# wpeebles/gangealing

Hardware: NVIDIA H100
Metric: gangealing_train_images_per_sec_256 (higher is better)
Workload: dtype f32

## Files before the change

gangealing_b200/_lib.py:

```python
import ctypes
import os

import torch

_HERE = os.path.dirname(os.path.abspath(__file__))
LIB_PATH = os.path.join(_HERE, "libgg_b200.so")

GG_F32, GG_F16, GG_BF16 = 0, 1, 2
PAD_MODES = {"zeros": 0, "border": 1, "reflection": 2}

_c = ctypes
_P, _I, _L, _F = _c.c_void_p, _c.c_int, _c.c_int64, _c.c_float

SIGNATURES = {
    "gg_version": (_I, []),
    "gg_last_error": (_c.c_char_p, []),
    "gg_sm_count": (_I, []),
    "gg_fused_bias_act": (_I, [_P, _P, _P, _P, _I, _I, _I, _F, _F, _L, _L, _L, _P]),
    "gg_noise_bias_act": (_I, [_P, _P, _P, _P, _P, _P, _I, _F, _F, _L, _L, _L, _P]),
    "gg_channel_scale_workspace": (_L, [_L, _L]),
    "gg_channel_scale": (_I, [_P, _P, _P, _P, _P, _P, _I, _L, _L, _P]),
    "gg_bias_act_backward_workspace": (_L, [_L, _L, _L]),
    "gg_bias_act_backward": (_I, [_P, _P, _P, _P, _P, _I, _F, _F, _L, _L, _L, _P]),
    "gg_upfirdn2d": (_I, [_P, _P, _P, _I, _L] + [_I] * 12 + [_P]),
    "gg_blur_noise_bias_act": (_I, [_P] * 7 + [_I, _L, _L] + [_I] * 9 + [_F, _F, _P]),
    "gg_mipmap_pyramid_elems": (_L, [_L, _I, _I, _I]),
    "gg_mipmap_build": (_I, [_P, _P, _I, _L, _I, _I, _I, _P]),
    "gg_mipmap_build_backward": (_I, [_P, _P, _L, _I, _I, _I, _P]),
    "gg_mipmap_warp_forward": (_I, [_P] * 5 + [_I, _L] + [_I] * 6 + [_F, _F, _I, _P]),
    "gg_warp_sample_indices": (_I, [_P, _P, _L, _I, _I, _I, _I, _F, _F, _I, _P]),
    "gg_stn_sample_forward": (_I, [_P] * 11 + [_I, _I, _L] + [_I] * 9 + [_F, _F, _I, _P]),
    "gg_mipmap_warp_lerp_forward": (_I, [_P] * 5 + [_L, _P, _P, _I, _I, _L] + [_I] * 6 + [_F, _F, _I, _P]),
    "gg_mipmap_warp_lerp_mean": (_I, [_P] * 4 + [_L, _P, _P, _I, _I, _L] + [_I] * 6 + [_F, _F, _I, _I, _P]),
    "gg_track_points_lerp": (_I, [_P] * 6 + [_I, _L, _L, _I, _I, _I, _P]),
    "gg_modconv_wsq": (_I, [_P, _P, _I, _I, _I, _P]),
    "gg_modconv_demod": (_I, [_P, _P, _P, _F, _F, _I, _I, _I, _P]),
    "gg_modconv_demod_batched": (_I, [_I, _P, _P, _P, _P, _P, _P, _F, _I, _P]),
    "gg_modconv_modulate": (_I, [_P, _P, _P, _P, _F, _I, _I, _I, _I, _I, _P]),
    "gg_noise_bias_act_nhwc": (_I, [_P] * 6 + [_I, _F, _F, _L, _I, _L, _P]),
    "gg_nhwc_rowwise_workspace": (_L, [_L, _I, _L]),
    "gg_channel_scale_nhwc": (_I, [_P] * 6 + [_I, _L, _I, _L, _P]),
    "gg_bias_act_backward_nhwc": (_I, [_P] * 5 + [_I, _F, _F, _L, _I, _L, _P]),
    "gg_blur_nhwc_workspace": (_L, [_I, _L] + [_I] * 9),
    "gg_blur_nhwc": (_I, [_P] * 12 + [_I, _L] + [_I] * 12 + [_F, _F, _P]),
    "gg_blur_nhwc_mask": (_I, [_P] * 9 + [_I, _L] + [_I] * 11 + [_F, _F, _P]),
    "gg_styled_tail_nhwc": (_I, [_P] * 12 + [_I, _I, _F, _F, _L, _I, _L, _P]),
    "gg_styled_tail_mask_nhwc": (_I, [_P] * 12 + [_I, _I, _F, _F, _L, _I, _L, _P]),
    "gg_styled_tail_backward_mask_nhwc": (_I, [_P] * 7 + [_I, _F, _F, _L, _I, _L, _P]),
    "gg_styled_tail_backward_workspace": (_L, [_I, _L, _I, _L]),
    "gg_styled_tail_backward_nhwc": (_I, [_P] * 12 + [_I, _F, _F, _L, _I, _L, _L, _P]),
    "gg_tent_downsample_forward": (_I, [_P] * 4 + [_L, _I, _I, _I, _I, _P]),
    "gg_tent_downsample_backward": (_I, [_P] * 4 + [_L, _I, _I, _I, _I, _P]),
    "gg_feature_distance_workspace": (_L, [_L, _I, _L]),
    "gg_feature_distance_forward": (_I, [_P] * 5 + [_I, _L, _I, _L, _F, _P]),
    "gg_feature_distance_backward": (_I, [_P] * 6 + [_I, _L, _I, _L, _F, _P]),
    "gg_bias_relu_pool_nhwc_forward": (_I, [_P, _P, _P, _P, _I, _L, _I, _I, _I, _P]),
    "gg_bias_relu_pool_nhwc_backward": (_I, [_P, _P, _P, _P, _I, _L, _I, _I, _I, _P]),
    "gg_to_rgb_nhwc_workspace": (_L, [_L, _I, _L]),
    "gg_to_rgb_nhwc_forward": (_I, [_P] * 5 + [_L, _I, _L, _P]),
    "gg_to_rgb_nhwc_backward": (_I, [_P] * 6 + [_L, _I, _L, _P]),
    "gg_nn_argmin_workspace": (_L, [_L, _L]),
    "gg_nn_argmin": (_I, [_P, _P, _P, _P, _L, _L, _I, _P]),
    "gg_splat2d_lookup_forward": (_I, [_P] * 8 + [_L, _L, _I, _I, _I, _I, _I, _F, _F, _I, _P]),
    "gg_scale_cast_multi": (_I, [_P, _P, _P, _I, _I, _P]),
    "gg_adam_ema_step": (_I, [_P, _P, _P, _I, _I, _P, _c.c_double, _c.c_double, _c.c_double, _c.c_double, _P]),
    "gg_tv_loss_workspace": (_L, [_L, _I, _I]),
    "gg_tv_loss_forward": (_I, [_P, _P, _P, _L, _I, _I, _P]),
    "gg_tv_loss_backward": (_I, [_P, _P, _P, _L, _I, _I, _P]),
    "gg_splat2d_workspace": (_L, [_L, _I, _I, _I]),
    "gg_splat2d_forward": (_I, [_P] * 6 + [_L, _L, _I, _I, _I, _I, _P]),
    "gg_splat_composite_grid_workspace": (_L, [_L, _L, _I, _I]),
    "gg_splat_composite_grid": (_I, [_P, _P, _L, _P, _P, _P, _P, _F, _F, _L, _L, _L, _I, _I, _I, _I, _I, _I, _P]),
    "gg_flow_compose_forward": (_I, [_P] * 7 + [_L, _I, _I, _I, _P]),
    "gg_flow_compose_backward": (_I, [_P] * 10 + [_L, _I, _I, _I, _P]),
    "gg_mipmap_warp_backward": (_I, [_P] * 7 + [_I, _L] + [_I] * 6 + [_F, _F, _I, _P]),
    "gg_laplacian_blend_workspace": (_L, [_L, _I, _I, _I, _I, _I]),
    "gg_laplacian_blend_forward": (_I, [_P] * 6 + [_L, _I, _I, _I, _I, _I, _P]),
    "gg_laplacian_blend_backward": (_I, [_P] * 9 + [_L, _I, _I, _I, _I, _I, _P]),
    "gg_tv_per_sample": (_I, [_P, _P, _L, _I, _I, _P]),
    "gg_pck_transfer_workspace": (_L, [_L, _L, _I]),
    "gg_pck_transfer": (_I, [_P] * 14 + [_L, _L, _I, _I, _I, _I, _I, _P]),
    "gg_batch_gram": (_I, [_P, _P, _P, _P, _L, _I, _P]),
    "gg_flow_image_grid": (_I, [_P, _P, _P, _L, _I, _I, _I, _I, _P]),
    "gg_image_grid": (_I, [_P, _P, _P, _L, _I, _I, _I, _I, _P]),
    "gg_cluster_accumulate": (_I, [_P] * 5 + [_L, _I, _I, _I, _I, _I] + [_L] * 6 + [_I, _P]),
}

_dll = None
CALLS = 0


def load():
    global _dll
    if _dll is None:
        if not os.path.exists(LIB_PATH):
            raise RuntimeError(
                "libgg_b200.so is missing (%s): build it with `python -m gangealing_b200.build` "
                "(there is no CPU/PyTorch fallback for these ops)" % LIB_PATH)
        dll = ctypes.CDLL(LIB_PATH)
        for name, (res, args) in SIGNATURES.items():
            fn = getattr(dll, name)
            fn.restype = res
            fn.argtypes = args
        _dll = dll
    return _dll


def check(rc, what):
    global CALLS
    CALLS += 1
    if rc != 0:
        msg = load().gg_last_error().decode("utf-8", "replace")
        raise RuntimeError("%s failed (%d): %s" % (what, rc, msg))


def dtype_code(t):
    d = t.dtype
    if d == torch.float32:
        return GG_F32
    if d == torch.float16:
        return GG_F16
    if d == torch.bfloat16:
        return GG_BF16
    raise RuntimeError("gangealing_b200: dtype %s is not supported (float32/float16/bfloat16)" % d)


def require_cuda(*tensors):
    for t in tensors:
        if t is None:
            continue
        if not t.is_cuda:
            raise RuntimeError("gangealing_b200 ops run on CUDA tensors only (got a %s tensor); "
                               "the CPU restatement lives in oracle/ and is test infrastructure" % t.device.type)
        if t.device.index != torch.cuda.current_device():
            raise RuntimeError("gangealing_b200: tensor lives on %s but the current device is cuda:%d; wrap the call in "
                               "`with torch.cuda.device(tensor.device):`" % (t.device, torch.cuda.current_device()))


def ptr(t):
    return None if t is None else t.data_ptr()


def is_nhwc(t):
    return (t.dim() == 4 and t.dtype in (torch.float32, torch.bfloat16) and t.shape[1] > 1 and t.shape[2] * t.shape[3] > 1
            and t.is_contiguous(memory_format=torch.channels_last) and not t.is_contiguous())


def nhwc_vec(t):
    return 8 if t.dtype == torch.bfloat16 else 4


def aligned16(t):
    return t.data_ptr() % 16 == 0


def dense_f32(t):
    if t.dtype != torch.float32 or not t.is_contiguous():
        t = t.float().contiguous()
    return t if aligned16(t) else t.clone()


def tensor_cache(t):
    stamp = (t._version, t.data_ptr(), t.device, t.dtype)
    ent = getattr(t, "_gg_cache", None)
    if ent is None or ent[0] != stamp:
        ent = (stamp, {})
        try:
            t._gg_cache = ent
        except Exception:
            pass
    return ent[1]


def filter_is_separable(kernel):
    memo = tensor_cache(kernel)
    v = memo.get("separable")
    if v is None:
        k = kernel.detach().float().cpu()
        big = k.abs().max()
        if big == 0:
            v = True
        else:
            i0, j0 = divmod(int(k.abs().argmax()), k.shape[1])
            v = bool((k - torch.outer(k[:, j0], k[i0, :]) / k[i0, j0]).abs().max() <= 1e-6 * big)
        memo["separable"] = v
    return v


def flipped_filter(kernel):
    memo = tensor_cache(kernel)
    f = memo.get("flipped")
    if f is None:
        f = torch.flip(kernel.detach(), [0, 1])
        fm = tensor_cache(f)
        fm["flipped"] = kernel.detach()
        if "separable" in memo:
            fm["separable"] = memo["separable"]
        memo["flipped"] = f
    return f


def invalidate(t):
    try:
        t._gg_cache = None
    except Exception:
        pass


def stream():
    return torch.cuda.current_stream().cuda_stream


def sm_count():
    return load().gg_sm_count()


def ship_table(slot, payload):
    capturing = torch.cuda.is_current_stream_capturing()
    ev = slot.get("event")
    if ev is not None and not capturing:
        ev.synchronize()
    slot["host"].copy_(payload)
    slot["dev"].copy_(slot["host"], non_blocking=True)
    if capturing:
        slot["event"] = None
    else:
        ev = torch.cuda.Event()
        ev.record()
        slot["event"] = ev
```

gangealing_b200/csrc/common.cuh:

```cuda
#pragma once
#include <cuda_bf16.h>
#include <cuda_fp16.h>
#include <cuda_runtime.h>
#include <stdint.h>

#include <cstdarg>
#include <cstdio>

#include "../../include/gg_b200.h"

namespace gg {

inline char* err_buf() {
  static thread_local char buf[512] = {0};
  return buf;
}
inline int fail(int code, const char* fmt, ...) {
  va_list ap;
  va_start(ap, fmt);
  vsnprintf(err_buf(), 512, fmt, ap);
  va_end(ap);
  return code;
}
inline int cuda_fail(cudaError_t e, const char* what) {
  return fail(GG_ERR_CUDA, "%s: %s", what, cudaGetErrorString(e));
}
#define GG_CHECK_LAUNCH(what)                               \
  do {                                                      \
    cudaError_t e__ = cudaPeekAtLastError();                \
    if (e__ != cudaSuccess) {                               \
      (void)cudaGetLastError();                             \
      return ::gg::cuda_fail(e__, what);                    \
    }                                                       \
  } while (0)

#define GG_DISPATCH_CASE_(code_, type_, ...) \
  case code_: { using T_ = type_; __VA_ARGS__; break; }
#define GG_DISPATCH_T(dtype_, who_, ...)                                                                             \
  switch (dtype_) {                                                                                                  \
    GG_DISPATCH_CASE_(GG_F32, float, __VA_ARGS__)                                                                    \
    GG_DISPATCH_CASE_(GG_BF16, __nv_bfloat16, __VA_ARGS__)                                                           \
    default: return ::gg::fail(GG_ERR_UNSUPPORTED, "%s: dtype %d not supported (fp32 or bf16)", who_, dtype_);       \
  }
#define GG_DISPATCH_T16(dtype_, who_, ...)                                                                           \
  switch (dtype_) {                                                                                                  \
    GG_DISPATCH_CASE_(GG_F32, float, __VA_ARGS__)                                                                    \
    GG_DISPATCH_CASE_(GG_F16, __half, __VA_ARGS__)                                                                   \
    GG_DISPATCH_CASE_(GG_BF16, __nv_bfloat16, __VA_ARGS__)                                                           \
    default: return ::gg::fail(GG_ERR_UNSUPPORTED, "%s: dtype %d not supported (fp32, fp16 or bf16)", who_, dtype_); \
  }

int sm_count();

inline bool aligned16(const void* p) { return (reinterpret_cast<uintptr_t>(p) & 15u) == 0; }
inline bool aligned8(const void* p) { return (reinterpret_cast<uintptr_t>(p) & 7u) == 0; }

struct DeviceOnce {
  unsigned long long mask[2] = {0ull, 0ull};
  int dev = 0;
  bool needed() {
    if (cudaGetDevice(&dev) != cudaSuccess || dev < 0 || dev >= 128) return true;
    return ((__atomic_load_n(&mask[dev >> 6], __ATOMIC_ACQUIRE) >> (dev & 63)) & 1ull) == 0ull;
  }
  void done() {
    if (dev >= 0 && dev < 128) __atomic_fetch_or(&mask[dev >> 6], 1ull << (dev & 63), __ATOMIC_RELEASE);
  }
};

template <typename T> struct Cvt;
template <> struct Cvt<float> {
  static __device__ __forceinline__ float to_f(float v) { return v; }
  static __device__ __forceinline__ float from_f(float v) { return v; }
};
template <> struct Cvt<__half> {
  static __device__ __forceinline__ float to_f(__half v) { return __half2float(v); }
  static __device__ __forceinline__ __half from_f(float v) { return __float2half_rn(v); }
};
template <> struct Cvt<__nv_bfloat16> {
  static __device__ __forceinline__ float to_f(__nv_bfloat16 v) { return __bfloat162float(v); }
  static __device__ __forceinline__ __nv_bfloat16 from_f(float v) { return __float2bfloat16_rn(v); }
};

template <typename T> struct alignas(16) Vec16 {
  static constexpr int N = 16 / sizeof(T);
  T v[N];
};

template <typename T>
__device__ __forceinline__ Vec16<T> ld_vec_stream(const T* p) {
  Vec16<T> r;
  uint4 u;
  asm volatile("ld.global.nc.L1::no_allocate.v4.u32 {%0,%1,%2,%3}, [%4];"
               : "=r"(u.x), "=r"(u.y), "=r"(u.z), "=r"(u.w)
               : "l"(p));
  *reinterpret_cast<uint4*>(&r) = u;
  return r;
}
template <typename T>
__device__ __forceinline__ void st_vec_stream(T* p, const Vec16<T>& r) {
  const uint4 u = *reinterpret_cast<const uint4*>(&r);
  asm volatile("st.global.L1::no_allocate.v4.u32 [%0], {%1,%2,%3,%4};" ::"l"(p), "r"(u.x), "r"(u.y),
               "r"(u.z), "r"(u.w)
               : "memory");
}

template <typename T> struct ChanVec;
template <> struct ChanVec<float> {
  static constexpr int V = 4;
  static __device__ __forceinline__ void unpack(const uint4& u, float (&f)[4]) {
    f[0] = __uint_as_float(u.x); f[1] = __uint_as_float(u.y); f[2] = __uint_as_float(u.z); f[3] = __uint_as_float(u.w);
  }
  static __device__ __forceinline__ uint4 pack(const float (&f)[4]) {
    return make_uint4(__float_as_uint(f[0]), __float_as_uint(f[1]), __float_as_uint(f[2]), __float_as_uint(f[3]));
  }
};
template <> struct ChanVec<__nv_bfloat16> {
  static constexpr int V = 8;
  static __device__ __forceinline__ void unpack(const uint4& u, float (&f)[8]) {
    f[0] = __uint_as_float(u.x << 16); f[1] = __uint_as_float(u.x & 0xffff0000u);
    f[2] = __uint_as_float(u.y << 16); f[3] = __uint_as_float(u.y & 0xffff0000u);
    f[4] = __uint_as_float(u.z << 16); f[5] = __uint_as_float(u.z & 0xffff0000u);
    f[6] = __uint_as_float(u.w << 16); f[7] = __uint_as_float(u.w & 0xffff0000u);
  }
  static __device__ __forceinline__ uint32_t pack2(float lo, float hi) {
    const __nv_bfloat162 h = __floats2bfloat162_rn(lo, hi);
    return *reinterpret_cast<const uint32_t*>(&h);
  }
  static __device__ __forceinline__ uint4 pack(const float (&f)[8]) {
    return make_uint4(pack2(f[0], f[1]), pack2(f[2], f[3]), pack2(f[4], f[5]), pack2(f[6], f[7]));
  }
};
__device__ __forceinline__ uint4 ldg_stream16(const void* p) {
  uint4 u;
  asm volatile("ld.global.nc.L1::no_allocate.v4.u32 {%0,%1,%2,%3}, [%4];" : "=r"(u.x), "=r"(u.y), "=r"(u.z), "=r"(u.w) : "l"(p));
  return u;
}
__device__ __forceinline__ void stg_stream16(void* p, const uint4& u) {
  asm volatile("st.global.L1::no_allocate.v4.u32 [%0], {%1,%2,%3,%4};" ::"l"(p), "r"(u.x), "r"(u.y), "r"(u.z), "r"(u.w) : "memory");
}

template <typename T> struct SignFloor { static constexpr float v = 0.f; };
template <> struct SignFloor<__nv_bfloat16> { static constexpr float v = 0x1p-134f; };

template <typename T, int V>
__device__ __forceinline__ uint32_t sign_bits(const float (&o)[V]) {
  uint32_t m = 0u;
#pragma unroll
  for (int k = 0; k < V; ++k) m |= (o[k] > SignFloor<T>::v ? 1u : 0u) << k;
  return m;
}
template <int V>
__device__ __forceinline__ uint32_t sign_word(uint32_t bits, int cq, unsigned lanes) {
  constexpr int L = 32 / V;
  uint32_t w = bits << (V * (cq & (L - 1)));
#pragma unroll
  for (int m = L / 2; m >= 1; m >>= 1) w |= __shfl_xor_sync(lanes, w, m);
  return w;
}
template <int V>
__device__ __forceinline__ uint32_t sign_load(const uint32_t* px, int cq) {
  return __ldg(px + (cq * V >> 5)) >> (cq * V & 31);
}

__device__ __forceinline__ float warp_sum(float v) {
#pragma unroll
  for (int o = 16; o > 0; o >>= 1) v += __shfl_xor_sync(0xffffffffu, v, o);
  return v;
}

__device__ __forceinline__ uint32_t smem_u32(const void* p) {
  return static_cast<uint32_t>(__cvta_generic_to_shared(p));
}
__device__ __forceinline__ void mbar_init(uint64_t* bar, uint32_t count) {
  asm volatile("mbarrier.init.shared::cta.b64 [%0], %1;" ::"r"(smem_u32(bar)), "r"(count));
}
__device__ __forceinline__ void mbar_fence_init() {
  asm volatile("fence.mbarrier_init.release.cluster;" ::: "memory");
}
__device__ __forceinline__ void mbar_expect_tx(uint64_t* bar, uint32_t bytes) {
  asm volatile("mbarrier.arrive.expect_tx.shared::cta.b64 _, [%0], %1;" ::"r"(smem_u32(bar)),
               "r"(bytes)
               : "memory");
}
__device__ __forceinline__ void mbar_wait(uint64_t* bar, uint32_t parity) {
  uint32_t done;
  uint32_t spins = 0;
  do {
    if (++spins == (1u << 28)) __trap();
    asm volatile(
        "{\n\t"
        ".reg .pred p;\n\t"
        "mbarrier.try_wait.parity.shared::cta.b64 p, [%1], %2;\n\t"
        "selp.u32 %0, 1, 0, p;\n\t"
        "}"
        : "=r"(done)
        : "r"(smem_u32(bar)), "r"(parity)
        : "memory");
  } while (!done);
}
__device__ __forceinline__ void tma_bulk_g2s(void* dst_smem, const void* src_gmem, uint32_t bytes,
                                             uint64_t* bar) {
  asm volatile(
      "cp.async.bulk.shared::cluster.global.mbarrier::complete_tx::bytes [%0], [%1], %2, [%3];" ::"r"(
          smem_u32(dst_smem)),
      "l"(src_gmem), "r"(bytes), "r"(smem_u32(bar))
      : "memory");
}

}
```

gangealing_b200/csrc/nhwc.cu:

```cuda
#include <cuda.h>

#include "common.cuh"
#include "nhwc_reduce.cuh"

namespace gg {
namespace {

constexpr int kT = 256;

template <typename T>
__global__ void __launch_bounds__(kT)
noise_bias_act_nhwc_kernel(T* __restrict__ out, const T* __restrict__ x, const float* __restrict__ noise,
                           const float* __restrict__ noise_weight, const float* __restrict__ bias,
                           const float* __restrict__ row_scale, float alpha, float gain, int64_t n_vec, int cv,
                           int64_t hw) {
  constexpr int V = ChanVec<T>::V;
  const float nw = noise ? (noise_weight ? __ldg(noise_weight) : 1.f) : 0.f;
  const int64_t base = (static_cast<int64_t>(blockIdx.x) * 4) * kT + threadIdx.x;
  uint4 xv[4];
#pragma unroll
  for (int u = 0; u < 4; ++u) {
    const int64_t v = base + static_cast<int64_t>(u) * kT;
    if (v < n_vec) xv[u] = ldg_stream16(x + v * V);
  }
#pragma unroll
  for (int u = 0; u < 4; ++u) {
    const int64_t v = base + static_cast<int64_t>(u) * kT;
    if (v < n_vec) {
      int64_t pix, n = 0;
      int cq;
      if (n_vec <= 0xffffffffLL) {
        const unsigned v32 = static_cast<unsigned>(v), p32 = v32 / static_cast<unsigned>(cv);
        cq = static_cast<int>(v32 - p32 * static_cast<unsigned>(cv));
        pix = p32;
        if (row_scale) n = p32 / static_cast<unsigned>(hw);
      } else {
        pix = v / cv;
        cq = static_cast<int>(v - pix * cv);
        if (row_scale) n = pix / hw;
      }
      const float nz = noise ? nw * __ldg(noise + pix) : 0.f;
      float xf[V], o[V];
      ChanVec<T>::unpack(xv[u], xf);
#pragma unroll
      for (int q = 0; q < V / 4; ++q) {
        const float4 b = bias ? __ldg(reinterpret_cast<const float4*>(bias) + cq * (V / 4) + q) : make_float4(0.f, 0.f, 0.f, 0.f);
        const float4 r = row_scale ? __ldg(reinterpret_cast<const float4*>(row_scale + n * cv * V) + cq * (V / 4) + q)
                                   : make_float4(1.f, 1.f, 1.f, 1.f);
        const float bb[4] = {b.x, b.y, b.z, b.w}, rr[4] = {r.x, r.y, r.z, r.w};
#pragma unroll
        for (int k = 0; k < 4; ++k) {
          const float t = fmaf(xf[4 * q + k], rr[k], bb[k]) + nz;
          o[4 * q + k] = (t > 0.f ? t : t * alpha) * gain;
        }
      }
      stg_stream16(out + v * V, ChanVec<T>::pack(o));
    }
  }
}

template <typename T, int MODE>
__global__ void __launch_bounds__(kT)
rowwise_nhwc_kernel(T* __restrict__ out, float* __restrict__ partial, const T* __restrict__ x,
                    const T* __restrict__ y, const float* __restrict__ s, float alpha, float gain, int cv,
                    int64_t hw, int chunk, int chunks_per_sample) {
  constexpr int V = ChanVec<T>::V;
  extern __shared__ float red[];
  const int64_t n = blockIdx.x / chunks_per_sample;
  const int ck = blockIdx.x - n * chunks_per_sample;
  const int64_t p0 = static_cast<int64_t>(ck) * chunk, p1 = min(p0 + chunk, hw);
  const int lanes_p = kT / cv > 0 ? kT / cv : 1;
  float acc[V];
#pragma unroll
  for (int k = 0; k < V; ++k) acc[k] = 0.f;
  const int cq = threadIdx.x % cv;
  const int pl = threadIdx.x / cv;
  if (pl < lanes_p) {
    float sv[V];
#pragma unroll
    for (int k = 0; k < V; ++k) sv[k] = (MODE == 0) ? __ldg(s + n * cv * V + cq * V + k) : 1.f;
    const bool has_y = (MODE == 1) || y != nullptr;
    auto body = [&](const uint4 xr, const uint4 yr, int64_t off) {
      float xf[V], yf[V], o[V];
      ChanVec<T>::unpack(xr, xf);
      ChanVec<T>::unpack(yr, yf);
#pragma unroll
      for (int k = 0; k < V; ++k) {
        if (MODE == 0) {
          o[k] = xf[k] * sv[k];
          if (has_y) acc[k] = fmaf(xf[k], yf[k], acc[k]);
        } else {
          o[k] = (yf[k] > 0.f ? xf[k] : xf[k] * alpha) * gain;
          acc[k] += o[k];
        }
      }
      *reinterpret_cast<uint4*>(out + off) = ChanVec<T>::pack(o);
    };
    const uint4 zero = make_uint4(0u, 0u, 0u, 0u);
    int64_t p = p0 + pl;
    for (; p + 3 * lanes_p < p1; p += 4 * lanes_p) {
      uint4 xv[4], yv[4];
      int64_t off[4];
#pragma unroll
      for (int u = 0; u < 4; ++u) {
        off[u] = ((n * hw + p + u * lanes_p) * cv + cq) * V;
        xv[u] = ldg_stream16(x + off[u]);
      }
#pragma unroll
      for (int u = 0; u < 4; ++u) yv[u] = has_y ? ldg_stream16(y + off[u]) : zero;
#pragma unroll
      for (int u = 0; u < 4; ++u) body(xv[u], yv[u], off[u]);
    }
    for (; p < p1; p += lanes_p) {
      const int64_t off = ((n * hw + p) * cv + cq) * V;
      const uint4 xv = ldg_stream16(x + off);
      const uint4 yv = has_y ? ldg_stream16(y + off) : zero;
      body(xv, yv, off);
    }
  }
  if (partial) {
    const int C = cv * V;
    if (pl < lanes_p) {
#pragma unroll
      for (int q = 0; q < V / 4; ++q)
        reinterpret_cast<float4*>(red + pl * C + cq * V)[q] = make_float4(acc[4 * q], acc[4 * q + 1], acc[4 * q + 2], acc[4 * q + 3]);
    }
    __syncthreads();
    for (int c = threadIdx.x; c < C; c += kT) {
      float t = 0.f;
      for (int l = 0; l < lanes_p; ++l) t += red[l * C + c];
      partial[static_cast<int64_t>(blockIdx.x) * C + c] = t;
    }
  }
}

__global__ void __launch_bounds__(kT)
to_rgb_nhwc_fwd_kernel(float* __restrict__ out, const float* __restrict__ x, const float* __restrict__ wm,
                       const float* __restrict__ bias, const float* __restrict__ skip, int c4, int64_t hw, int chunk,
                       int chunks_per_sample) {
  extern __shared__ __align__(16) float wsm[];
  const int64_t n = blockIdx.x / chunks_per_sample;
  const int ck = blockIdx.x - n * chunks_per_sample;
  const int64_t p0 = static_cast<int64_t>(ck) * chunk, p1 = min(p0 + chunk, hw);
  {
    const float4* src = reinterpret_cast<const float4*>(wm + n * 3 * c4 * 4);
    float4* dst = reinterpret_cast<float4*>(wsm);
    for (int i = threadIdx.x; i < 3 * c4; i += kT) dst[i] = __ldg(src + i);
  }
  __syncthreads();
  const float4* w4 = reinterpret_cast<const float4*>(wsm);
  const int l = threadIdx.x & 7, grp = threadIdx.x >> 3;
  const bool vec_ok = (hw & 3) == 0;
  const unsigned gmask = 0xffu << (threadIdx.x & 24);
  for (int64_t pb = p0 + grp * 4; pb < p1; pb += (kT / 8) * 4) {
    float acc[4][3];
#pragma unroll
    for (int u = 0; u < 4; ++u) acc[u][0] = acc[u][1] = acc[u][2] = 0.f;
    const float4* xp[4];
#pragma unroll
    for (int u = 0; u < 4; ++u) {
      const int64_t pu = min(pb + u, p1 - 1);
      xp[u] = reinterpret_cast<const float4*>(x + (n * hw + pu) * c4 * 4);
    }
    for (int q = l; q < c4; q += 8) {
      float4 xv[4];
#pragma unroll
      for (int u = 0; u < 4; ++u) xv[u] = __ldcs(xp[u] + q);
      const float4 w0 = w4[q], w1 = w4[c4 + q], w2 = w4[2 * c4 + q];
#pragma unroll
      for (int u = 0; u < 4; ++u) {
        acc[u][0] = fmaf(xv[u].x, w0.x, fmaf(xv[u].y, w0.y, fmaf(xv[u].z, w0.z, fmaf(xv[u].w, w0.w, acc[u][0]))));
        acc[u][1] = fmaf(xv[u].x, w1.x, fmaf(xv[u].y, w1.y, fmaf(xv[u].z, w1.z, fmaf(xv[u].w, w1.w, acc[u][1]))));
        acc[u][2] = fmaf(xv[u].x, w2.x, fmaf(xv[u].y, w2.y, fmaf(xv[u].z, w2.z, fmaf(xv[u].w, w2.w, acc[u][2]))));
      }
    }
#pragma unroll
    for (int m = 4; m >= 1; m >>= 1)
#pragma unroll
      for (int u = 0; u < 4; ++u)
#pragma unroll
        for (int o = 0; o < 3; ++o) acc[u][o] += __shfl_xor_sync(gmask, acc[u][o], m);
    if (l < 3) {
      const int o = l;
      float r[4];
#pragma unroll
      for (int u = 0; u < 4; ++u) r[u] = (o == 0 ? acc[u][0] : o == 1 ? acc[u][1] : acc[u][2]) + (bias ? __ldg(bias + o) : 0.f);
      const int64_t off = (n * 3 + o) * hw + pb;
      if (vec_ok && pb + 3 < p1) {
        if (skip) {
          const float4 sk = __ldg(reinterpret_cast<const float4*>(skip + off));
          r[0] += sk.x; r[1] += sk.y; r[2] += sk.z; r[3] += sk.w;
        }
        *reinterpret_cast<float4*>(out + off) = make_float4(r[0], r[1], r[2], r[3]);
      } else {
#pragma unroll
        for (int u = 0; u < 4; ++u)
          if (pb + u < p1) out[off + u] = r[u] + (skip ? __ldg(skip + off + u) : 0.f);
      }
    }
  }
}

__global__ void __launch_bounds__(kT)
to_rgb_nhwc_bwd_kernel(float* __restrict__ gx, float* __restrict__ partial, const float* __restrict__ g,
                       const float* __restrict__ x, const float* __restrict__ wm, int c4, int64_t hw, int chunk,
                       int chunks_per_sample) {
  extern __shared__ float red[];
  const int64_t n = blockIdx.x / chunks_per_sample;
  const int ck = blockIdx.x - n * chunks_per_sample;
  const int64_t p0 = static_cast<int64_t>(ck) * chunk, p1 = min(p0 + chunk, hw);
  const int lanes_p = kT / c4 > 0 ? kT / c4 : 1;
  const int cq = threadIdx.x % c4, pl = threadIdx.x / c4;
  float4 a0 = make_float4(0.f, 0.f, 0.f, 0.f), a1 = a0, a2 = a0;
  if (pl < lanes_p) {
    const float4* wp = reinterpret_cast<const float4*>(wm + n * 3 * c4 * 4);
    const float4 w0 = __ldg(wp + cq), w1 = __ldg(wp + c4 + cq), w2 = __ldg(wp + 2 * c4 + cq);
    const float* g0 = g + n * 3 * hw;
    auto body = [&](int64_t p, const float4 xv, float s0, float s1, float s2) {
      float4 o;
      o.x = fmaf(w2.x, s2, fmaf(w1.x, s1, w0.x * s0)); o.y = fmaf(w2.y, s2, fmaf(w1.y, s1, w0.y * s0));
      o.z = fmaf(w2.z, s2, fmaf(w1.z, s1, w0.z * s0)); o.w = fmaf(w2.w, s2, fmaf(w1.w, s1, w0.w * s0));
      if (gx) *reinterpret_cast<float4*>(gx + ((n * hw + p) * c4 + cq) * 4) = o;
      a0.x = fmaf(s0, xv.x, a0.x); a0.y = fmaf(s0, xv.y, a0.y); a0.z = fmaf(s0, xv.z, a0.z); a0.w = fmaf(s0, xv.w, a0.w);
      a1.x = fmaf(s1, xv.x, a1.x); a1.y = fmaf(s1, xv.y, a1.y); a1.z = fmaf(s1, xv.z, a1.z); a1.w = fmaf(s1, xv.w, a1.w);
      a2.x = fmaf(s2, xv.x, a2.x); a2.y = fmaf(s2, xv.y, a2.y); a2.z = fmaf(s2, xv.z, a2.z); a2.w = fmaf(s2, xv.w, a2.w);
    };
    const float4 zero = make_float4(0.f, 0.f, 0.f, 0.f);
    int64_t p = p0 + pl;
    for (; p + 3 * lanes_p < p1; p += 4 * lanes_p) {
      float4 xv[4];
      float s[4][3];
#pragma unroll
      for (int u = 0; u < 4; ++u) {
        const int64_t pu = p + u * lanes_p;
        xv[u] = partial ? __ldcs(reinterpret_cast<const float4*>(x + ((n * hw + pu) * c4 + cq) * 4)) : zero;
        s[u][0] = __ldg(g0 + pu); s[u][1] = __ldg(g0 + hw + pu); s[u][2] = __ldg(g0 + 2 * hw + pu);
      }
#pragma unroll
      for (int u = 0; u < 4; ++u) body(p + u * lanes_p, xv[u], s[u][0], s[u][1], s[u][2]);
    }
    for (; p < p1; p += lanes_p) {
      const float4 xv = partial ? __ldcs(reinterpret_cast<const float4*>(x + ((n * hw + p) * c4 + cq) * 4)) : zero;
      body(p, xv, __ldg(g0 + p), __ldg(g0 + hw + p), __ldg(g0 + 2 * hw + p));
    }
  }
  if (partial) {
    float4* r4 = reinterpret_cast<float4*>(red);
    if (pl < lanes_p) {
      r4[(pl * 3 + 0) * c4 + cq] = a0; r4[(pl * 3 + 1) * c4 + cq] = a1; r4[(pl * 3 + 2) * c4 + cq] = a2;
    }
    __syncthreads();
    for (int i = threadIdx.x; i < 3 * c4; i += kT) {
      float4 t = make_float4(0.f, 0.f, 0.f, 0.f);
      for (int q = 0; q < lanes_p; ++q) {
        const float4 v = r4[q * 3 * c4 + i];
        t.x += v.x; t.y += v.y; t.z += v.z; t.w += v.w;
      }
      reinterpret_cast<float4*>(partial + static_cast<int64_t>(blockIdx.x) * 3 * c4 * 4)[i] = t;
    }
  }
}

template <typename T> struct BlurGeom {
  static constexpr int V = ChanVec<T>::V;
  static constexpr int CB = 8 * V;
  static constexpr int COLS = (V == 4) ? 2 : 1;
  static constexpr int BX = 32 * COLS;
  static constexpr int TW = BX + 3;
  static constexpr int STAGE_ELEMS = 4 * TW * CB;
};
constexpr int kRY = 4;
constexpr int kNS = 3;

struct BlurNhwcParams {
  int n, c, in_h, in_w, out_h, out_w;
  int pad_x0, pad_y0;
  int seg_rows;
  int act;
  float alpha, gain;
};

__device__ __forceinline__ void tma_load_4d(void* smem_dst, const CUtensorMap* tmap, int c0, int x0, int y0, int n0,
                                            uint64_t* bar) {
  asm volatile(
      "cp.async.bulk.tensor.4d.shared::cluster.global.tile.mbarrier::complete_tx::bytes [%0], [%1, {%2, %3, %4, %5}], [%6];"
      ::"r"(smem_u32(smem_dst)), "l"(tmap), "r"(c0), "r"(x0), "r"(y0), "r"(n0), "r"(smem_u32(bar))
      : "memory");
}

template <typename T, int MODE, bool SEP, bool FAST = false>
__global__ void __launch_bounds__(kT, 2)
blur_nhwc_kernel(T* __restrict__ out, T* __restrict__ out2, const __grid_constant__ CUtensorMap tmap,
                 const float* __restrict__ filt, int kh, int kw, const float* __restrict__ noise,
                 const float* __restrict__ noise_weight, const float* __restrict__ bias,
                 const float* __restrict__ row_scale, const float* __restrict__ scale2, const T* __restrict__ mul,
                 float* __restrict__ partial, BlurNhwcParams p) {
  using G = BlurGeom<T>;
  constexpr int V = G::V, CB = G::CB, COLS = G::COLS, BX = G::BX, TW = G::TW;
  constexpr bool FUSED = MODE == 1 || MODE == 3;
  constexpr bool MASK = MODE == 3;
  extern __shared__ __align__(128) unsigned char tiles_raw[];
  T* tiles = reinterpret_cast<T*>(tiles_raw);
  __shared__ uint64_t full_bar[kNS];
  const int tid = threadIdx.x;
  const int cq = tid & 7;
  const int xg = tid >> 3;
  const int chunks = p.c / CB;
  const int bx = blockIdx.x / chunks, cc = blockIdx.x - bx * chunks;
  const int n = blockIdx.z;
  const int oy0 = blockIdx.y * p.seg_rows;
  const int rows_out = min(p.seg_rows, p.out_h - oy0);
  const int x_out0 = bx * BX;
  const int c0 = cc * CB;
  const int iy0 = oy0 - p.pad_y0, ix0 = x_out0 - p.pad_x0;
  const int rows_in = rows_out + 3;
  const int n_stage_iters = (rows_in + kRY - 1) / kRY;
  constexpr uint32_t kStageBytes = G::STAGE_ELEMS * sizeof(T);

  if (tid == 0) {
#pragma unroll
    for (int s = 0; s < kNS; ++s) mbar_init(&full_bar[s], 1);
    mbar_fence_init();
  }
  __syncthreads();
  if (tid == 0) {
#pragma unroll
    for (int s = 0; s < kNS - 1; ++s)
      if (s < n_stage_iters) {
        mbar_expect_tx(&full_bar[s], kStageBytes);
        tma_load_4d(tiles + s * G::STAGE_ELEMS, &tmap, c0, ix0, iy0 + s * kRY, n, &full_bar[s]);
      }
  }

  float kf[4][4];
#pragma unroll
  for (int a = 0; a < 4; ++a)
#pragma unroll
    for (int b = 0; b < 4; ++b)
      kf[a][b] = (a < kh && b < kw) ? __ldg(filt + (kh - 1 - a) * kw + (kw - 1 - b)) : 0.f;
  float ku[4], kv[4];
  {
    int a0 = 0, b0 = 0;
    float big = 0.f;
#pragma unroll
    for (int a = 0; a < 4; ++a)
#pragma unroll
      for (int b = 0; b < 4; ++b)
        if (fabsf(kf[a][b]) > big) { big = fabsf(kf[a][b]); a0 = a; b0 = b; }
    float piv = 1.f;
#pragma unroll
    for (int a = 0; a < 4; ++a)
#pragma unroll
      for (int b = 0; b < 4; ++b)
        if (a == a0 && b == b0) piv = kf[a][b];
    const float inv = big > 0.f ? 1.f / piv : 0.f;
#pragma unroll
    for (int a = 0; a < 4; ++a) {
      float col = 0.f;
#pragma unroll
      for (int b = 0; b < 4; ++b) if (b == b0) col = kf[a][b];
      ku[a] = col * inv;
    }
#pragma unroll
    for (int b = 0; b < 4; ++b) {
      float row = 0.f;
#pragma unroll
      for (int a = 0; a < 4; ++a) if (a == a0) row = kf[a][b];
      kv[b] = row;
    }
  }

  float bq[V], rq[V], sq[V], dacc[V];
#pragma unroll
  for (int k = 0; k < V; ++k) { bq[k] = 0.f; rq[k] = 1.f; sq[k] = 1.f; dacc[k] = 0.f; }
  float nw = 0.f;
  const int64_t nc0 = static_cast<int64_t>(n) * p.c + c0 + cq * V;
  if (MODE != 0) {
    if (row_scale) {
#pragma unroll
      for (int k = 0; k < V; ++k) rq[k] = __ldg(row_scale + nc0 + k);
    }
  }
  if (FUSED) {
    if (bias) {
#pragma unroll
      for (int k = 0; k < V; ++k) bq[k] = __ldg(bias + c0 + cq * V + k);
    }
    if (scale2) {
#pragma unroll
      for (int k = 0; k < V; ++k) sq[k] = __ldg(scale2 + nc0 + k);
    }
    nw = noise ? (noise_weight ? __ldg(noise_weight) : 1.f) : 0.f;
  }
  constexpr bool fast = FUSED && FAST;
  const float neg = (p.act == 3) ? p.alpha : 1.f;
  if (fast) {
#pragma unroll
    for (int k = 0; k < V; ++k) { rq[k] *= p.gain; bq[k] *= p.gain; }
    nw *= p.gain;
  }
  const int xo = x_out0 + COLS * xg;
  const int64_t row_stride = static_cast<int64_t>(p.out_w) * p.c;
  const int64_t obase = ((static_cast<int64_t>(n) * p.out_h + oy0) * p.out_w + xo) * p.c + c0 + cq * V;
  int64_t ocur = obase - 3 * row_stride;
  bool okc[COLS];
#pragma unroll
  for (int j = 0; j < COLS; ++j) okc[j] = xo + j < p.out_w;
  float nzn[kRY][COLS];
#pragma unroll
  for (int rr = 0; rr < kRY; ++rr)
#pragma unroll
    for (int j = 0; j < COLS; ++j) nzn[rr][j] = 0.f;
  const float* noise_base = noise ? noise + (static_cast<int64_t>(n) * p.out_h + oy0) * p.out_w + xo : nullptr;
  auto fetch_noise = [&](int it_) {
#pragma unroll
    for (int rr = 0; rr < kRY; ++rr) {
      const int ro = it_ * kRY + rr - 3;
#pragma unroll
      for (int j = 0; j < COLS; ++j) nzn[rr][j] = 0.f;
      if (ro >= 0 && ro < rows_out) {
        const float* np_ = noise_base + static_cast<int64_t>(ro) * p.out_w;
#pragma unroll
        for (int j = 0; j < COLS; ++j)
          if (okc[j]) nzn[rr][j] = __ldg(np_ + j);
      }
    }
  };
  if (FUSED && noise) fetch_noise(0);

  uint4 mcur[COLS], mnext[COLS];
#pragma unroll
  for (int j = 0; j < COLS; ++j) mcur[j] = mnext[j] = make_uint4(0u, 0u, 0u, 0u);
  auto fetch_mul = [&](int ro_) {
    if (ro_ >= 0 && ro_ < rows_out) {
      const int64_t mo = obase + ro_ * row_stride;
#pragma unroll
      for (int j = 0; j < COLS; ++j)
        if (okc[j]) mnext[j] = __ldg(reinterpret_cast<const uint4*>(mul + mo + static_cast<int64_t>(j) * p.c));
    }
  };
  if (MODE == 2 && mul) { fetch_mul(-3 + 3); }

  float hwin[SEP ? 4 : 1][COLS][V];
  float rwin[SEP ? 1 : 4][COLS + 3][V];
  int r_in = 0;
  for (int it = 0; it < n_stage_iters; ++it) {
    const int stage = it % kNS;
    if (tid == 0) {
      const int nxt = it + kNS - 1;
      if (nxt < n_stage_iters) {
        const int ns = nxt % kNS;
        asm volatile("fence.proxy.async.shared::cta;" ::: "memory");
        mbar_expect_tx(&full_bar[ns], kStageBytes);
        tma_load_4d(tiles + ns * G::STAGE_ELEMS, &tmap, c0, ix0, iy0 + nxt * kRY, n, &full_bar[ns]);
      }
    }
    float nzc[kRY][COLS];
#pragma unroll
    for (int rr = 0; rr < kRY; ++rr)
#pragma unroll
      for (int j = 0; j < COLS; ++j) nzc[rr][j] = nzn[rr][j];
    if (FUSED && noise && it + 1 < n_stage_iters) fetch_noise(it + 1);
    if (MODE == 2 && mul && it + 1 < n_stage_iters) {
#pragma unroll
      for (int rr = 0; rr < kRY; ++rr) {
        const int ro = (it + 1) * kRY + rr - 3;
        if (ro >= 0 && ro < rows_out) {
          const T* mp = mul + obase + ro * row_stride;
#pragma unroll
          for (int j = 0; j < COLS; ++j)
            if (okc[j]) asm volatile("prefetch.global.L2 [%0];" ::"l"(mp + static_cast<int64_t>(j) * p.c));
        }
      }
    }
    mbar_wait(&full_bar[stage], static_cast<uint32_t>((it / kNS) & 1));
    const T* st = tiles + stage * G::STAGE_ELEMS;
#pragma unroll
    for (int rr = 0; rr < kRY; ++rr, ++r_in, ocur += row_stride) {
      if (MODE == 2 && mul) {
#pragma unroll
        for (int j = 0; j < COLS; ++j) mcur[j] = mnext[j];
        fetch_mul(r_in - 3 + 1);
      }
      const uint4* rowp = reinterpret_cast<const uint4*>(st + (rr * TW + COLS * xg) * CB) + cq;
      float q[COLS + 3][V];
#pragma unroll
      for (int i = 0; i < COLS + 3; ++i) ChanVec<T>::unpack(rowp[i * 8], q[i]);
      if constexpr (SEP) {
#pragma unroll
        for (int j = 0; j < COLS; ++j)
#pragma unroll
          for (int k = 0; k < V; ++k) {
            float h = __fmul_rn(kv[0], q[j][k]);
            h = __fmaf_rn(kv[1], q[j + 1][k], h);
            h = __fmaf_rn(kv[2], q[j + 2][k], h);
            h = __fmaf_rn(kv[3], q[j + 3][k], h);
            hwin[rr][j][k] = h;
          }
      } else {
#pragma unroll
        for (int i = 0; i < COLS + 3; ++i)
#pragma unroll
          for (int k = 0; k < V; ++k) rwin[rr][i][k] = q[i][k];
      }
      const int ro = r_in - 3;
      if (ro >= 0 && ro < rows_out) {
#pragma unroll
        for (int j = 0; j < COLS; ++j) {
          float a4[V];
          if constexpr (SEP) {
#pragma unroll
            for (int k = 0; k < V; ++k) {
              float a = __fmul_rn(ku[0], hwin[(rr + 1) & 3][j][k]);
              a = __fmaf_rn(ku[1], hwin[(rr + 2) & 3][j][k], a);
              a = __fmaf_rn(ku[2], hwin[(rr + 3) & 3][j][k], a);
              a = __fmaf_rn(ku[3], hwin[rr][j][k], a);
              a4[k] = a;
            }
          } else {
#pragma unroll
            for (int k = 0; k < V; ++k) a4[k] = 0.f;
#pragma unroll
            for (int a = 0; a < 4; ++a)
#pragma unroll
              for (int b = 0; b < 4; ++b)
#pragma unroll
                for (int k = 0; k < V; ++k) a4[k] = fmaf(kf[a][b], rwin[(rr + 1 + a) & 3][j + b][k], a4[k]);
          }
          const int64_t ooff = ocur + j * p.c;
          if (FUSED) {
            const float nzj = nw * nzc[rr][j];
            float o2[V];
#pragma unroll
            for (int k = 0; k < V; ++k) {
              float t = __fmaf_rn(a4[k], rq[k], __fadd_rn(bq[k], nzj));
              const float tn = __fmul_rn(t, neg);
              if (fast) t = fmaxf(t, tn);
              else t = (t > 0.f ? t : tn) * p.gain;
              a4[k] = t;
              o2[k] = __fmul_rn(t, sq[k]);
            }
            uint32_t word = 0u;
            if (MASK) word = sign_word<V>(sign_bits<T>(a4), cq, 0xffffffffu);
            if (okc[j]) {
              if (MASK) {
                if ((cq * V & 31) == 0) reinterpret_cast<uint32_t*>(out)[ooff >> 5] = word;
              } else if (out) {
                *reinterpret_cast<uint4*>(out + ooff) = ChanVec<T>::pack(a4);
              }
              if (out2) *reinterpret_cast<uint4*>(out2 + ooff) = ChanVec<T>::pack(o2);
            }
          } else if (MODE == 2) {
            if (okc[j]) {
              if (mul) {
                float mf[V];
                ChanVec<T>::unpack(mcur[j], mf);
#pragma unroll
                for (int k = 0; k < V; ++k) dacc[k] = fmaf(a4[k], mf[k], dacc[k]);
              }
#pragma unroll
              for (int k = 0; k < V; ++k) a4[k] *= rq[k];
              *reinterpret_cast<uint4*>(out + ooff) = ChanVec<T>::pack(a4);
            }
          } else {
            if (okc[j]) *reinterpret_cast<uint4*>(out + ooff) = ChanVec<T>::pack(a4);
          }
        }
      }
    }
    __syncthreads();
  }
  if (MODE == 2 && partial) {
    float* red = reinterpret_cast<float*>(tiles_raw);
#pragma unroll
    for (int k = 0; k < V; ++k) red[xg * CB + cq * V + k] = dacc[k];
    __syncthreads();
    if (tid < CB) {
      float t = 0.f;
#pragma unroll 8
      for (int g = 0; g < 32; ++g) t += red[g * CB + tid];
      const int64_t K = static_cast<int64_t>(gridDim.x / chunks) * gridDim.y;
      const int64_t kidx = static_cast<int64_t>(bx) * gridDim.y + blockIdx.y;
      partial[(static_cast<int64_t>(n) * K + kidx) * p.c + c0 + tid] = t;
    }
  }
}

typedef CUresult (*EncodeTiledFn)(CUtensorMap*, CUtensorMapDataType, cuuint32_t, void*, const cuuint64_t*, const cuuint64_t*,
                                  const cuuint32_t*, const cuuint32_t*, CUtensorMapInterleave, CUtensorMapSwizzle,
                                  CUtensorMapL2promotion, CUtensorMapFloatOOBfill);

inline EncodeTiledFn encode_fn() {
  static EncodeTiledFn fn = nullptr;
  if (!fn) {
    void* p = nullptr;
    cudaDriverEntryPointQueryResult q;
    if (cudaGetDriverEntryPoint("cuTensorMapEncodeTiled", &p, cudaEnableDefault, &q) == cudaSuccess &&
        q == cudaDriverEntryPointSuccess)
      fn = reinterpret_cast<EncodeTiledFn>(p);
  }
  return fn;
}

inline int grid1(int64_t total, int per_cta) {
  int64_t g = (total + per_cta - 1) / per_cta;
  return static_cast<int>(g > 0 ? g : 1);
}

}
}

using namespace gg;

extern "C" {

static inline int vec_of(int dtype) { return dtype == GG_BF16 ? 8 : 4; }

int gg_noise_bias_act_nhwc(void* out, const void* x, const float* noise, const float* noise_weight, const float* bias,
                           const float* row_scale, int dtype, float alpha, float scale, int64_t N, int C, int64_t HW,
                           void* stream) {
  if (N < 0 || C < 0 || HW < 0) return fail(GG_ERR_BAD_ARG, "noise_bias_act_nhwc: negative size");
  if (dtype != GG_F32 && dtype != GG_BF16) return fail(GG_ERR_UNSUPPORTED, "noise_bias_act_nhwc: dtype %d not supported", dtype);
  const int64_t numel = N * HW * C;
  if (numel == 0) return GG_OK;
  const int V = vec_of(dtype);
  if (C % V != 0) return fail(GG_ERR_UNSUPPORTED, "noise_bias_act_nhwc: C must be a multiple of %d", V);
  if (!out || !x) return fail(GG_ERR_BAD_ARG, "noise_bias_act_nhwc: null tensor");
  if (!aligned16(bias) || !aligned16(row_scale))
    return fail(GG_ERR_BAD_ARG, "noise_bias_act_nhwc: bias and row_scale must be 16-byte aligned");
  const int64_t n_vec = numel / V;
  const int64_t grid = (n_vec + 4 * kT - 1) / (4 * kT);
  if (grid > 0x7fffffffLL) return fail(GG_ERR_BAD_ARG, "noise_bias_act_nhwc: tensor too large");
  GG_DISPATCH_T(dtype, "noise_bias_act_nhwc",
                (noise_bias_act_nhwc_kernel<T_><<<static_cast<unsigned>(grid), kT, 0, static_cast<cudaStream_t>(stream)>>>(
                    static_cast<T_*>(out), static_cast<const T_*>(x), noise, noise_weight, bias, row_scale, alpha, scale,
                    n_vec, C / V, HW)));
  GG_CHECK_LAUNCH("noise_bias_act_nhwc launch");
  return GG_OK;
}

static int64_t rowwise_chunk(int64_t N, int cv, int64_t HW) {
  const int lanes_p = kT / cv > 0 ? kT / cv : 1;
  const int64_t target = 8LL * sm_count();
  int64_t k = (target + N - 1) / N;
  const int64_t kmax = (HW + 4 * lanes_p - 1) / (4 * lanes_p);
  if (k > kmax) k = kmax;
  if (k < 1) k = 1;
  return (HW + k - 1) / k;
}

int64_t gg_nhwc_rowwise_workspace(int64_t N, int C, int64_t HW) {
  if (N <= 0 || C <= 0 || HW <= 0 || C % 4 != 0) return 0;
  const int64_t chunk = rowwise_chunk(N, C / 4, HW);
  const int64_t chunk8 = (C % 8 == 0) ? rowwise_chunk(N, C / 8, HW) : chunk;
  const int64_t k = (HW + (chunk < chunk8 ? chunk : chunk8) - 1) / (chunk < chunk8 ? chunk : chunk8);
  return N * k * C * static_cast<int64_t>(sizeof(float));
}

static int launch_rowwise(int mode, void* out, float* dst, void* workspace, const void* x, const void* y, const float* s,
                          int dtype, float alpha, float gain, int64_t N, int C, int64_t HW, bool per_sample, void* stream) {
  if (N < 0 || C < 0 || HW < 0) return fail(GG_ERR_BAD_ARG, "nhwc rowwise: negative size");
  if (dtype != GG_F32 && dtype != GG_BF16) return fail(GG_ERR_UNSUPPORTED, "nhwc rowwise: dtype %d not supported", dtype);
  if (N * HW * C == 0) {
    const int64_t sums = (per_sample ? N : 1) * C;
    if (dst && sums > 0) {
      cudaError_t e = cudaMemsetAsync(dst, 0, sums * sizeof(float), static_cast<cudaStream_t>(stream));
      if (e != cudaSuccess) return cuda_fail(e, "nhwc rowwise memset");
    }
    return GG_OK;
  }
  const int V = vec_of(dtype);
  if (C % V != 0 || C / V > kT) return fail(GG_ERR_UNSUPPORTED, "nhwc rowwise: C must be a multiple of %d and <= %d", V, V * kT);
  if (!out || !x) return fail(GG_ERR_BAD_ARG, "nhwc rowwise: null tensor");
  if (dst && !workspace) return fail(GG_ERR_BAD_ARG, "nhwc rowwise: reduction needs a workspace");
  const int cv = C / V;
  const int64_t chunk64 = rowwise_chunk(N, cv, HW);
  if (chunk64 > 0x7fffffffLL) return fail(GG_ERR_BAD_ARG, "nhwc rowwise: plane too large");
  const int chunk = static_cast<int>(chunk64);
  const int K = static_cast<int>((HW + chunk - 1) / chunk);
  const int64_t grid = N * K;
  if (grid > 0x7fffffffLL) return fail(GG_ERR_BAD_ARG, "nhwc rowwise: too many CTAs");
  const int lanes_p = kT / cv > 0 ? kT / cv : 1;
  const size_t smem = static_cast<size_t>(lanes_p) * C * sizeof(float);
  float* partial = dst ? static_cast<float*>(workspace) : nullptr;
  auto st = static_cast<cudaStream_t>(stream);
  const unsigned g = static_cast<unsigned>(grid);
  if (mode == 0) {
    GG_DISPATCH_T(dtype, "nhwc rowwise",
                  (rowwise_nhwc_kernel<T_, 0><<<g, kT, smem, st>>>(static_cast<T_*>(out), partial, static_cast<const T_*>(x),
                                                                 dst ? static_cast<const T_*>(y) : nullptr, s, alpha, gain,
                                                                 cv, HW, chunk, K)));
  } else {
    GG_DISPATCH_T(dtype, "nhwc rowwise",
                  (rowwise_nhwc_kernel<T_, 1><<<g, kT, smem, st>>>(static_cast<T_*>(out), partial, static_cast<const T_*>(x),
                                                                 static_cast<const T_*>(y), s, alpha, gain, cv, HW, chunk, K)));
  }
  GG_CHECK_LAUNCH("nhwc rowwise launch");
  if (dst) {
    const int64_t rows = per_sample ? N : 1;
    const int kk = per_sample ? K : static_cast<int>(N * K);
    nhwc_finish_kernel<<<static_cast<unsigned>(rows * ((C + 31) / 32)), dim3(32, 32), 0, st>>>(dst, partial, rows, kk, C);
    GG_CHECK_LAUNCH("nhwc finish launch");
  }
  return GG_OK;
}

int gg_channel_scale_nhwc(void* out, float* row_dot, void* workspace, const void* x, const void* y, const float* s,
                          int dtype, int64_t N, int C, int64_t HW, void* stream) {
  if (!s) return fail(GG_ERR_BAD_ARG, "channel_scale_nhwc: null scale");
  if (row_dot && !y) return fail(GG_ERR_BAD_ARG, "channel_scale_nhwc: row_dot needs y");
  return launch_rowwise(0, out, row_dot, workspace, x, y, s, dtype, 0.f, 1.f, N, C, HW, true, stream);
}

int gg_bias_act_backward_nhwc(void* gx, float* grad_bias, void* workspace, const void* g, const void* out_saved,
                              int dtype, float alpha, float scale, int64_t N, int C, int64_t HW, void* stream) {
  if (!out_saved) return fail(GG_ERR_BAD_ARG, "bias_act_backward_nhwc: null saved output");
  return launch_rowwise(1, gx, grad_bias, workspace, g, out_saved, nullptr, dtype, alpha, scale, N, C, HW, false, stream);
}

int64_t gg_to_rgb_nhwc_workspace(int64_t N, int C, int64_t HW) { return 3 * gg_nhwc_rowwise_workspace(N, C, HW); }

int gg_to_rgb_nhwc_forward(float* out, const float* x, const float* wm, const float* bias, const float* skip, int64_t N,
                           int C, int64_t HW, void* stream) {
  if (N < 0 || C < 0 || HW < 0) return fail(GG_ERR_BAD_ARG, "to_rgb_nhwc: negative size");
  if (N * HW == 0) return GG_OK;
  if (C < 32 || C % 32 != 0 || C > 1024) return fail(GG_ERR_UNSUPPORTED, "to_rgb_nhwc: C must be a multiple of 32, <= 1024");
  if (!out || !x || !wm) return fail(GG_ERR_BAD_ARG, "to_rgb_nhwc: null tensor");
  if (!aligned16(wm) || (HW % 4 == 0 && (!aligned16(skip) || !aligned16(out))))
    return fail(GG_ERR_BAD_ARG, "to_rgb_nhwc: wm (and skip, out when HW %% 4 == 0) must be 16-byte aligned");
  const int64_t target = 8LL * sm_count();
  int64_t k = (target + N - 1) / N;
  const int64_t kmax = (HW + 127) / 128;
  if (k > kmax) k = kmax;
  if (k < 1) k = 1;
  int64_t chunk = ((HW + k - 1) / k + 127) / 128 * 128;
  if (chunk > 0x7fffff00LL) return fail(GG_ERR_BAD_ARG, "to_rgb_nhwc: plane too large");
  const int K = static_cast<int>((HW + chunk - 1) / chunk);
  const int64_t grid = N * K;
  if (grid > 0x7fffffffLL) return fail(GG_ERR_BAD_ARG, "to_rgb_nhwc: too many CTAs");
  to_rgb_nhwc_fwd_kernel<<<static_cast<unsigned>(grid), kT, static_cast<size_t>(3) * C * sizeof(float),
                           static_cast<cudaStream_t>(stream)>>>(out, x, wm, bias, skip, C / 4, HW, static_cast<int>(chunk), K);
  GG_CHECK_LAUNCH("to_rgb_nhwc forward launch");
  return GG_OK;
}

int gg_to_rgb_nhwc_backward(float* gx, float* gwm, void* workspace, const float* g, const float* x, const float* wm,
                            int64_t N, int C, int64_t HW, void* stream) {
  if (N < 0 || C < 0 || HW < 0) return fail(GG_ERR_BAD_ARG, "to_rgb_nhwc backward: negative size");
  if (N * HW == 0 || C == 0) {
    if (gwm && N * C > 0) {
      cudaError_t e = cudaMemsetAsync(gwm, 0, N * 3 * C * sizeof(float), static_cast<cudaStream_t>(stream));
      if (e != cudaSuccess) return cuda_fail(e, "to_rgb_nhwc backward memset");
    }
    return GG_OK;
  }
  if (C % 4 != 0 || C > 1024) return fail(GG_ERR_UNSUPPORTED, "to_rgb_nhwc backward: C must be a multiple of 4, <= 1024");
  if (!g || !wm || (!gx && !gwm)) return fail(GG_ERR_BAD_ARG, "to_rgb_nhwc backward: null tensor");
  if (gwm && (!x || !workspace)) return fail(GG_ERR_BAD_ARG, "to_rgb_nhwc backward: gwm needs x and a workspace");
  if (!aligned16(wm)) return fail(GG_ERR_BAD_ARG, "to_rgb_nhwc backward: wm must be 16-byte aligned");
  const int c4 = C / 4;
  const int64_t chunk64 = rowwise_chunk(N, c4, HW);
  if (chunk64 > 0x7fffffffLL) return fail(GG_ERR_BAD_ARG, "to_rgb_nhwc backward: plane too large");
  const int chunk = static_cast<int>(chunk64);
  const int K = static_cast<int>((HW + chunk - 1) / chunk);
  const int64_t grid = N * K;
  if (grid > 0x7fffffffLL) return fail(GG_ERR_BAD_ARG, "to_rgb_nhwc backward: too many CTAs");
  const int lanes_p = kT / c4 > 0 ? kT / c4 : 1;
  const size_t smem = static_cast<size_t>(lanes_p) * 3 * C * sizeof(float);
  auto st = static_cast<cudaStream_t>(stream);
  float* partial = gwm ? static_cast<float*>(workspace) : nullptr;
  to_rgb_nhwc_bwd_kernel<<<static_cast<unsigned>(grid), kT, smem, st>>>(gx, partial, g, x, wm, c4, HW, chunk, K);
  GG_CHECK_LAUNCH("to_rgb_nhwc backward launch");
  if (gwm) {
    nhwc_finish_kernel<<<static_cast<unsigned>(N * ((3 * C + 31) / 32)), dim3(32, 32), 0, st>>>(gwm, partial, N, K, 3 * C);
    GG_CHECK_LAUNCH("to_rgb_nhwc finish launch");
  }
  return GG_OK;
}

struct BlurPlan {
  int out_h, out_w, xblocks, chunks, segs, seg_rows;
};
static int blur_plan(BlurPlan* pl, int dtype, int64_t N, int C, int in_h, int in_w, int kernel_h, int kernel_w, int pad_x0,
                     int pad_x1, int pad_y0, int pad_y1) {
  const int V = vec_of(dtype);
  const int CB = 8 * V, BX = (V == 4) ? 64 : 32;
  if (C % CB != 0) return fail(GG_ERR_UNSUPPORTED, "blur_nhwc: C must be a multiple of %d", CB);
  pl->out_h = in_h + pad_y0 + pad_y1 - kernel_h + 1;
  pl->out_w = in_w + pad_x0 + pad_x1 - kernel_w + 1;
  if (pl->out_h < 1 || pl->out_w < 1) return fail(GG_ERR_BAD_ARG, "blur_nhwc: empty output");
  pl->xblocks = (pl->out_w + BX - 1) / BX;
  pl->chunks = C / CB;
  const int64_t base_ctas = static_cast<int64_t>(pl->xblocks) * pl->chunks * (N > 0 ? N : 1);
  int segs = static_cast<int>((2LL * 2 * sm_count() + base_ctas - 1) / base_ctas);
  int seg_rows = (pl->out_h + segs - 1) / segs;
  if (seg_rows < 16) seg_rows = pl->out_h < 16 ? pl->out_h : 16;
  seg_rows = (seg_rows + 3) / 4 * 4;
  pl->seg_rows = seg_rows;
  pl->segs = (pl->out_h + seg_rows - 1) / seg_rows;
  return GG_OK;
}

int64_t gg_blur_nhwc_workspace(int dtype, int64_t N, int C, int in_h, int in_w, int kernel_h, int kernel_w, int pad_x0,
                               int pad_x1, int pad_y0, int pad_y1) {
  BlurPlan pl;
  if (N <= 0 || C <= 0 || (dtype != GG_F32 && dtype != GG_BF16)) return 0;
  if (blur_plan(&pl, dtype, N, C, in_h, in_w, kernel_h, kernel_w, pad_x0, pad_x1, pad_y0, pad_y1) != GG_OK) return 0;
  return N * static_cast<int64_t>(pl.xblocks) * pl.segs * C * static_cast<int64_t>(sizeof(float));
}

}

template <typename T>
static int launch_blur(void* out, void* out2, const void* in, const float* kernel, const float* noise,
                       const float* noise_weight, const float* bias, const float* row_scale, const float* scale2,
                       const void* mul, float* row_dot, void* workspace, int64_t N, int C, int in_h, int in_w, int kernel_h,
                       int kernel_w, int separable, int pad_x0, int pad_x1, int pad_y0, int pad_y1, int mode, int act,
                       float alpha, float scale, void* stream, int dtype, bool out_is_mask) {
  using G = BlurGeom<T>;
  BlurPlan pl;
  int rc = blur_plan(&pl, dtype, N, C, in_h, in_w, kernel_h, kernel_w, pad_x0, pad_x1, pad_y0, pad_y1);
  if (rc != GG_OK) return rc;
  EncodeTiledFn enc = encode_fn();
  if (!enc) return fail(GG_ERR_CUDA, "blur_nhwc: cuTensorMapEncodeTiled is not available from this driver");
  struct MapKey { const void* ptr; int64_t n; int c, h, w, es; };
  struct MapEnt { MapKey key; CUtensorMap map; bool valid; };
  static thread_local MapEnt cache[16] = {};
  static thread_local unsigned cache_next = 0;
  const MapKey key = {in, N, C, in_h, in_w, static_cast<int>(sizeof(T))};
  const CUtensorMap* cached = nullptr;
  for (int i = 0; i < 16 && !cached; ++i)
    if (cache[i].valid && cache[i].key.ptr == key.ptr && cache[i].key.n == key.n && cache[i].key.c == key.c &&
        cache[i].key.h == key.h && cache[i].key.w == key.w && cache[i].key.es == key.es)
      cached = &cache[i].map;
  CUtensorMap tmap;
  if (cached) tmap = *cached;
  const cuuint64_t es = sizeof(T);
  const cuuint64_t gdim[4] = {static_cast<cuuint64_t>(C), static_cast<cuuint64_t>(in_w), static_cast<cuuint64_t>(in_h),
                              static_cast<cuuint64_t>(N)};
  const cuuint64_t gstr[3] = {static_cast<cuuint64_t>(C) * es, static_cast<cuuint64_t>(in_w) * C * es,
                              static_cast<cuuint64_t>(in_h) * in_w * C * es};
  const cuuint32_t box[4] = {G::CB, G::TW, kRY, 1};
  const cuuint32_t estr[4] = {1, 1, 1, 1};
  if (!cached) {
    const CUresult r = enc(&tmap, sizeof(T) == 4 ? CU_TENSOR_MAP_DATA_TYPE_FLOAT32 : CU_TENSOR_MAP_DATA_TYPE_BFLOAT16, 4,
                           const_cast<void*>(in), gdim, gstr, box, estr, CU_TENSOR_MAP_INTERLEAVE_NONE,
                           CU_TENSOR_MAP_SWIZZLE_NONE, CU_TENSOR_MAP_L2_PROMOTION_L2_128B, CU_TENSOR_MAP_FLOAT_OOB_FILL_NONE);
    if (r != CUDA_SUCCESS) return fail(GG_ERR_CUDA, "blur_nhwc: cuTensorMapEncodeTiled failed (%d)", static_cast<int>(r));
    MapEnt& e = cache[cache_next++ % 16];
    e.key = key; e.map = tmap; e.valid = true;
  }
  BlurNhwcParams p;
  p.n = static_cast<int>(N); p.c = C; p.in_h = in_h; p.in_w = in_w; p.out_h = pl.out_h; p.out_w = pl.out_w;
  p.pad_x0 = pad_x0; p.pad_y0 = pad_y0;
  p.act = act; p.alpha = alpha; p.gain = scale;
  p.seg_rows = pl.seg_rows;
  const dim3 grid(static_cast<unsigned>(pl.xblocks * pl.chunks), static_cast<unsigned>(pl.segs), static_cast<unsigned>(N));
  const size_t smem = static_cast<size_t>(kNS) * G::STAGE_ELEMS * sizeof(T);
  static DeviceOnce configured;
  if (configured.needed()) {
    cudaError_t e = cudaSuccess;
    const void* kernels[12] = {reinterpret_cast<const void*>(blur_nhwc_kernel<T, 0, true>),
                              reinterpret_cast<const void*>(blur_nhwc_kernel<T, 0, false>),
                              reinterpret_cast<const void*>(blur_nhwc_kernel<T, 1, true, false>),
                              reinterpret_cast<const void*>(blur_nhwc_kernel<T, 1, false, false>),
                              reinterpret_cast<const void*>(blur_nhwc_kernel<T, 1, true, true>),
                              reinterpret_cast<const void*>(blur_nhwc_kernel<T, 1, false, true>),
                              reinterpret_cast<const void*>(blur_nhwc_kernel<T, 3, true, false>),
                              reinterpret_cast<const void*>(blur_nhwc_kernel<T, 3, false, false>),
                              reinterpret_cast<const void*>(blur_nhwc_kernel<T, 3, true, true>),
                              reinterpret_cast<const void*>(blur_nhwc_kernel<T, 3, false, true>),
                              reinterpret_cast<const void*>(blur_nhwc_kernel<T, 2, true>),
                              reinterpret_cast<const void*>(blur_nhwc_kernel<T, 2, false>)};
    for (int i = 0; i < 12 && e == cudaSuccess; ++i)
      e = cudaFuncSetAttribute(kernels[i], cudaFuncAttributeMaxDynamicSharedMemorySize, static_cast<int>(smem));
    if (e != cudaSuccess) return cuda_fail(e, "blur_nhwc smem opt-in");
    configured.done();
  }
  auto st = static_cast<cudaStream_t>(stream);
  float* partial = (mode == 2 && row_dot) ? static_cast<float*>(workspace) : nullptr;
  const bool fast = scale > 0.f && ((act == 3 && alpha >= 0.f && alpha <= 1.f) || act == 1);
#define GG_BLUR(M_, S_, F_)                                                                                          \
  blur_nhwc_kernel<T, M_, S_, F_><<<grid, kT, smem, st>>>(static_cast<T*>(out), static_cast<T*>(out2), tmap, kernel, kernel_h, \
                                                         kernel_w, noise, noise_weight, bias, row_scale, scale2,     \
                                                         static_cast<const T*>(mul), partial, p)
  if (mode == 1 && out_is_mask) {
    if (fast) { if (separable) GG_BLUR(3, true, true); else GG_BLUR(3, false, true); }
    else { if (separable) GG_BLUR(3, true, false); else GG_BLUR(3, false, false); }
  }
  else if (mode == 1) {
    if (fast) { if (separable) GG_BLUR(1, true, true); else GG_BLUR(1, false, true); }
    else { if (separable) GG_BLUR(1, true, false); else GG_BLUR(1, false, false); }
  }
  else if (mode == 2) { if (separable) GG_BLUR(2, true, false); else GG_BLUR(2, false, false); }
  else { if (separable) GG_BLUR(0, true, false); else GG_BLUR(0, false, false); }
#undef GG_BLUR
  GG_CHECK_LAUNCH("blur_nhwc launch");
  if (partial) {
    const int K = pl.xblocks * pl.segs;
    nhwc_finish_kernel<<<static_cast<unsigned>(N * ((C + 31) / 32)), dim3(32, 32), 0, st>>>(row_dot, partial, N, K, C);
    GG_CHECK_LAUNCH("blur_nhwc finish launch");
  }
  return GG_OK;
}

extern "C" {

int gg_blur_nhwc(void* out, void* out2, const void* in, const float* kernel, const float* noise, const float* noise_weight,
                 const float* bias, const float* row_scale, const float* scale2, const void* mul, float* row_dot,
                 void* workspace, int dtype, int64_t N, int C, int in_h, int in_w, int kernel_h, int kernel_w, int separable,
                 int pad_x0, int pad_x1, int pad_y0, int pad_y1, int mode, int act, float alpha, float scale, void* stream) {
  if (N < 0 || C < 0 || in_h < 1 || in_w < 1) return fail(GG_ERR_BAD_ARG, "blur_nhwc: bad shape");
  if (kernel_h < 1 || kernel_w < 1 || kernel_h > 4 || kernel_w > 4) return fail(GG_ERR_UNSUPPORTED, "blur_nhwc: filter must be <= 4x4");
  if (mode < 0 || mode > 2) return fail(GG_ERR_BAD_ARG, "blur_nhwc: mode must be 0 (blur), 1 (fused tail) or 2 (adjoint epilogue)");
  if (act != 1 && act != 3) return fail(GG_ERR_UNSUPPORTED, "blur_nhwc: act must be 1 or 3");
  if (dtype != GG_F32 && dtype != GG_BF16) return fail(GG_ERR_UNSUPPORTED, "blur_nhwc: dtype %d not supported (fp32 or bf16)", dtype);
  if (N == 0 || C == 0) return GG_OK;
  if (!in || !kernel) return fail(GG_ERR_BAD_ARG, "blur_nhwc: null tensor");
  if (mode == 1 ? (!out && !out2) : !out) return fail(GG_ERR_BAD_ARG, "blur_nhwc: null output");
  if (mode != 1 && out2) return fail(GG_ERR_BAD_ARG, "blur_nhwc: out2 belongs to the fused tail (mode 1)");
  if (mode == 2 && row_dot && (!mul || !workspace)) return fail(GG_ERR_BAD_ARG, "blur_nhwc: row_dot needs `mul` and a workspace");
  if (N > 65535) return fail(GG_ERR_UNSUPPORTED, "blur_nhwc: batch > 65535");
  if (mode == 0) { noise = nullptr; noise_weight = nullptr; bias = nullptr; row_scale = nullptr; scale2 = nullptr; }
  GG_DISPATCH_T(dtype, "blur_nhwc",
                return launch_blur<T_>(out, out2, in, kernel, noise, noise_weight, bias, row_scale, scale2, mul, row_dot,
                                       workspace, N, C, in_h, in_w, kernel_h, kernel_w, separable, pad_x0, pad_x1, pad_y0,
                                       pad_y1, mode, act, alpha, scale, stream, dtype, false));
  return GG_OK;
}

int gg_blur_nhwc_mask(void* mask, void* out2, const void* in, const float* kernel, const float* noise,
                      const float* noise_weight, const float* bias, const float* row_scale, const float* scale2, int dtype,
                      int64_t N, int C, int in_h, int in_w, int kernel_h, int kernel_w, int separable, int pad_x0, int pad_x1,
                      int pad_y0, int pad_y1, int act, float alpha, float scale, void* stream) {
  if (N < 0 || C < 0 || in_h < 1 || in_w < 1) return fail(GG_ERR_BAD_ARG, "blur_nhwc_mask: bad shape");
  if (kernel_h < 1 || kernel_w < 1 || kernel_h > 4 || kernel_w > 4) return fail(GG_ERR_UNSUPPORTED, "blur_nhwc_mask: filter must be <= 4x4");
  if (act != 1 && act != 3) return fail(GG_ERR_UNSUPPORTED, "blur_nhwc_mask: act must be 1 or 3");
  if (dtype != GG_F32 && dtype != GG_BF16) return fail(GG_ERR_UNSUPPORTED, "blur_nhwc_mask: dtype %d not supported (fp32 or bf16)", dtype);
  if (N == 0 || C == 0) return GG_OK;
  if (!in || !kernel) return fail(GG_ERR_BAD_ARG, "blur_nhwc_mask: null tensor");
  if (!mask) return fail(GG_ERR_BAD_ARG, "blur_nhwc_mask: null mask");
  if (out2 && !scale2) return fail(GG_ERR_BAD_ARG, "blur_nhwc_mask: out2 needs scale2");
  if (N > 65535) return fail(GG_ERR_UNSUPPORTED, "blur_nhwc_mask: batch > 65535");
  GG_DISPATCH_T(dtype, "blur_nhwc_mask",
                return launch_blur<T_>(mask, out2, in, kernel, noise, noise_weight, bias, row_scale, scale2, nullptr, nullptr,
                                       nullptr, N, C, in_h, in_w, kernel_h, kernel_w, separable, pad_x0, pad_x1, pad_y0,
                                       pad_y1, 1, act, alpha, scale, stream, dtype, true));
  return GG_OK;
}

}
```

gangealing_b200/op/nhwc.py:

```python
import torch

from .. import _lib

CL = torch.channels_last

TIMING = None


def elementwise_ok(t):
    return _lib.is_nhwc(t) and t.shape[1] % _lib.nhwc_vec(t) == 0 and _lib.aligned16(t)


def rowwise_ok(t):
    return elementwise_ok(t) and t.shape[1] // _lib.nhwc_vec(t) <= 256


def blur_ok(t, kh, kw, up=(1, 1), down=(1, 1)):
    return (_lib.is_nhwc(t) and t.shape[1] % (8 * _lib.nhwc_vec(t)) == 0 and kh <= 4 and kw <= 4
            and up == (1, 1) and down == (1, 1) and _lib.aligned16(t))


def _f32(t, numel=None):
    if t is None:
        return None
    t = _lib.dense_f32(t.detach())
    if numel is not None and t.numel() != numel:
        raise RuntimeError("channels-last op: expected %d fp32 values, got %d" % (numel, t.numel()))
    return t


def noise_plane(noise, n, h, w):
    if noise is None:
        return None
    noise = noise.detach()
    if noise.numel() != n * h * w:
        noise = noise.expand(n, 1, h, w)
    return noise.float().contiguous()


def sign_mask_empty(n, c, h, w, device):
    if c % 32:
        raise RuntimeError("sign mask: C = %d is not a multiple of 32" % c)
    return torch.empty((n, h, w, c // 32), dtype=torch.int32, device=device)


def blur(x, kernel, pad, mode=0, noise=None, noise_weight=None, bias=None, row_scale=None, scale2=None, want_out=True,
         want_out2=False, mul=None, want_dot=False, negative_slope=0.2, gain=1.0, act=3, want_mask=False):
    n, c, in_h, in_w = x.shape
    taps = kernel.detach()
    if taps.dtype != torch.float32 or not taps.is_contiguous():
        taps = taps.float().contiguous()
    kh, kw = taps.shape
    out_h = in_h + pad[2] + pad[3] - kh + 1
    out_w = in_w + pad[0] + pad[1] - kw + 1
    if out_h < 1 or out_w < 1:
        raise RuntimeError("blur: empty output (%d x %d)" % (out_h, out_w))
    lib = _lib.load()
    code = _lib.dtype_code(x)

    def empty():
        return torch.empty((n, c, out_h, out_w), dtype=x.dtype, device=x.device, memory_format=CL)
    if want_mask and mode != 1:
        raise RuntimeError("blur: the sign mask belongs to the fused tail (mode 1)")
    if want_mask:
        out = sign_mask_empty(n, c, out_h, out_w, x.device)
    else:
        out = empty() if (want_out or mode != 1) else None
    out2 = empty() if (mode == 1 and want_out2) else None
    nz = noise_plane(noise, n, out_h, out_w) if mode == 1 else None
    dot = ws = None
    if mode == 2 and want_dot:
        if (mul is None or mul.shape != (n, c, out_h, out_w) or mul.dtype != x.dtype or not mul.is_contiguous(memory_format=CL)
                or not _lib.aligned16(mul)):
            raise RuntimeError("blur (adjoint epilogue): `mul` must be a 16-byte-aligned channels-last tensor of the output's "
                               "shape and dtype")
        dot = torch.empty((n, c), dtype=torch.float32, device=x.device)
        nbytes = lib.gg_blur_nhwc_workspace(code, n, c, in_h, in_w, kh, kw, pad[0], pad[1], pad[2], pad[3])
        ws = torch.empty(max(1, nbytes // 4), dtype=torch.float32, device=x.device)
    timed = TIMING is not None and mode == 1
    if timed:
        ev0, ev1 = torch.cuda.Event(enable_timing=True), torch.cuda.Event(enable_timing=True)
        ev0.record()
    nw, b, rs, s2 = _f32(noise_weight, 1), _f32(bias, c), _f32(row_scale, n * c), _f32(scale2, n * c)
    sep = 1 if _lib.filter_is_separable(kernel) else 0
    if want_mask:
        rc = lib.gg_blur_nhwc_mask(out.data_ptr(), _lib.ptr(out2), x.data_ptr(), taps.data_ptr(), _lib.ptr(nz), _lib.ptr(nw),
                                   _lib.ptr(b), _lib.ptr(rs), _lib.ptr(s2), code, n, c, in_h, in_w, kh, kw, sep, pad[0],
                                   pad[1], pad[2], pad[3], act, negative_slope, gain, _lib.stream())
    else:
        rc = lib.gg_blur_nhwc(_lib.ptr(out), _lib.ptr(out2), x.data_ptr(), taps.data_ptr(), _lib.ptr(nz),
                              _lib.ptr(nw), _lib.ptr(b), _lib.ptr(rs),
                              _lib.ptr(s2), _lib.ptr(mul if dot is not None else None), _lib.ptr(dot), _lib.ptr(ws),
                              code, n, c, in_h, in_w, kh, kw, sep, pad[0], pad[1],
                              pad[2], pad[3], mode, act, negative_slope, gain, _lib.stream())
    _lib.check(rc, "gg_blur_nhwc_mask" if want_mask else "gg_blur_nhwc")
    if timed:
        ev1.record()
        es = x.element_size()
        writes = (out is not None and not want_mask) + (out2 is not None)
        TIMING.append((ev0, ev1, es * n * c * (in_h * in_w + writes * out_h * out_w) + (4 * n * out_h * out_w if nz is not None else 0)
                       + (out.numel() * 4 if want_mask else 0)
                       + 4 * ((2 + (scale2 is not None)) * c + 1 + kh * kw)))
    return out, out2, dot


def noise_bias_act(x, noise, noise_weight, bias, row_scale, negative_slope, gain):
    n, c, h, w = x.shape
    out = torch.empty_like(x)
    nz, nw, b, rs = noise_plane(noise, n, h, w), _f32(noise_weight, 1), _f32(bias, c), _f32(row_scale, n * c)
    rc = _lib.load().gg_noise_bias_act_nhwc(out.data_ptr(), x.data_ptr(), _lib.ptr(nz), _lib.ptr(nw), _lib.ptr(b),
                                            _lib.ptr(rs), _lib.dtype_code(x), negative_slope, gain, n, c, h * w,
                                            _lib.stream())
    _lib.check(rc, "gg_noise_bias_act_nhwc")
    return out


def bias_act_backward(g, out_saved, negative_slope, gain, want_bias_grad):
    n, c, h, w = out_saved.shape
    lib = _lib.load()
    gx = torch.empty_like(out_saved)
    grad_bias = ws = None
    if want_bias_grad:
        grad_bias = torch.empty(c, dtype=torch.float32, device=g.device)
        ws = torch.empty(max(1, lib.gg_nhwc_rowwise_workspace(n, c, h * w) // 4), dtype=torch.float32, device=g.device)
    rc = lib.gg_bias_act_backward_nhwc(gx.data_ptr(), _lib.ptr(grad_bias), _lib.ptr(ws), g.data_ptr(), out_saved.data_ptr(),
                                       _lib.dtype_code(out_saved), negative_slope, gain, n, c, h * w, _lib.stream())
    _lib.check(rc, "gg_bias_act_backward_nhwc")
    return gx, grad_bias


def channel_scale(x, s, y=None):
    n, c, h, w = x.shape
    lib = _lib.load()
    out = torch.empty_like(x)
    dot = ws = None
    if y is not None:
        dot = torch.empty((n, c), dtype=torch.float32, device=x.device)
        ws = torch.empty(max(1, lib.gg_nhwc_rowwise_workspace(n, c, h * w) // 4), dtype=torch.float32, device=x.device)
    sc = _f32(s, n * c)
    rc = lib.gg_channel_scale_nhwc(out.data_ptr(), _lib.ptr(dot), _lib.ptr(ws), x.data_ptr(), _lib.ptr(y), sc.data_ptr(),
                                   _lib.dtype_code(x), n, c, h * w, _lib.stream())
    _lib.check(rc, "gg_channel_scale_nhwc")
    return out, dot


def _activation_like(t, like, who, name):
    if t is not None and (t.shape != like.shape or t.dtype != like.dtype or not t.is_contiguous(memory_format=CL)
                          or not _lib.aligned16(t)):
        raise RuntimeError("%s: %s must be a 16-byte-aligned channels-last tensor of the activation's shape and dtype"
                           % (who, name))


def _rgb_grad_ok(g_rgb, n, h, w, who):
    if g_rgb is not None and (g_rgb.shape != (n, 3, h, w) or g_rgb.dtype != torch.float32 or not g_rgb.is_contiguous()):
        raise RuntimeError("%s: g_rgb must be a dense fp32 (N, 3, H, W) tensor" % who)


def styled_tail(raw, noise, noise_weight, bias, demod, s_next, wm, rgb_bias, skip, want_out, negative_slope, gain, act=3,
                want_mask=False):
    _activation_like(raw, raw, "styled_tail", "raw")
    n, c, h, w = raw.shape
    if want_mask:
        out = sign_mask_empty(n, c, h, w, raw.device)
    else:
        out = torch.empty_like(raw) if want_out else None
    xs = torch.empty_like(raw) if s_next is not None else None
    rgb = torch.empty((n, 3, h, w), dtype=torch.float32, device=raw.device) if wm is not None else None
    sk = None
    if skip is not None and rgb is not None:
        sk = skip.detach()
        if sk.dtype != torch.float32 or not sk.is_contiguous():
            sk = sk.float().contiguous()
        if sk.shape != rgb.shape:
            raise RuntimeError("styled_tail: skip must be (N, 3, H, W)")
    consts = [noise_plane(noise, n, h, w), _f32(noise_weight, 1), _f32(bias, c), _f32(demod, n * c), _f32(s_next, n * c),
              _f32(wm, n * 3 * c), _f32(rgb_bias, 3)]
    lib = _lib.load()
    entry = lib.gg_styled_tail_mask_nhwc if want_mask else lib.gg_styled_tail_nhwc
    rc = entry(_lib.ptr(out), _lib.ptr(xs), _lib.ptr(rgb), raw.data_ptr(), *[_lib.ptr(t) for t in consts], _lib.ptr(sk),
               _lib.dtype_code(raw), act, negative_slope, gain, n, c, h * w, _lib.stream())
    _lib.check(rc, "gg_styled_tail_mask_nhwc" if want_mask else "gg_styled_tail_nhwc")
    return out, xs, rgb


def styled_tail_backward(g_xs, g_rgb, out_saved, raw, s_next, demod, wm, want_ds, want_dd, want_dwm, negative_slope, gain):
    n, c, h, w = out_saved.shape
    lib = _lib.load()
    dev = out_saved.device
    want_ds = want_ds and g_xs is not None
    want_dd = want_dd and raw is not None
    want_dwm = want_dwm and g_rgb is not None
    for name, t in (("out_saved", out_saved), ("g_xs", g_xs), ("raw", raw if want_dd else None)):
        _activation_like(t, out_saved, "styled_tail_backward", name)
    _rgb_grad_ok(g_rgb, n, h, w, "styled_tail_backward")
    g_raw = torch.empty_like(out_saved)
    rows = int(want_ds) + int(want_dd) + 3 * int(want_dwm)
    block = torch.empty((n, rows, c), dtype=torch.float32, device=dev) if rows else None
    r = 0
    d_s = d_d = d_w = None
    if want_ds:
        d_s = block[:, r]; r += 1
    if want_dd:
        d_d = block[:, r]; r += 1
    if want_dwm:
        d_w = block[:, r:r + 3]
    code = _lib.dtype_code(out_saved)
    ws = None
    if rows:
        ws = torch.empty(max(1, lib.gg_styled_tail_backward_workspace(code, n, c, h * w) // 4), dtype=torch.float32, device=dev)
    consts = [_f32(s_next, n * c), _f32(demod, n * c), _f32(wm, n * 3 * c)]
    rc = lib.gg_styled_tail_backward_nhwc(g_raw.data_ptr(), _lib.ptr(d_s), _lib.ptr(d_d), _lib.ptr(d_w), _lib.ptr(ws),
                                          _lib.ptr(g_xs), _lib.ptr(g_rgb), out_saved.data_ptr(),
                                          _lib.ptr(raw if want_dd else None),
                                          *[_lib.ptr(t) for t in consts],
                                          code, negative_slope, gain, n, c, h * w, rows * c, _lib.stream())
    _lib.check(rc, "gg_styled_tail_backward_nhwc")
    return g_raw, d_s, d_d, d_w


def styled_tail_backward_mask(g_xs, g_rgb, mask, s_next, demod, wm, negative_slope, gain, dtype):
    n, h, w, words = mask.shape
    c = 32 * words
    g_raw = torch.empty((n, c, h, w), dtype=dtype, device=mask.device, memory_format=CL)
    _activation_like(g_xs, g_raw, "styled_tail_backward_mask", "g_xs")
    _rgb_grad_ok(g_rgb, n, h, w, "styled_tail_backward_mask")
    consts = [_f32(s_next, n * c), _f32(demod, n * c), _f32(wm, n * 3 * c)]
    rc = _lib.load().gg_styled_tail_backward_mask_nhwc(g_raw.data_ptr(), _lib.ptr(g_xs), _lib.ptr(g_rgb), mask.data_ptr(),
                                                       *[_lib.ptr(t) for t in consts], _lib.dtype_code(g_raw),
                                                       negative_slope, gain, n, c, h * w, _lib.stream())
    _lib.check(rc, "gg_styled_tail_backward_mask_nhwc")
    return g_raw
```

gangealing_b200/stylegan2/networks.py:

```python
import math
import random

import torch
from torch import nn
from torch.nn import functional as F

from ..opset import cuda_ops


def make_kernel(k):
    k = torch.tensor(k, dtype=torch.float32)
    if k.ndim == 1:
        k = k[None, :] * k[:, None]
    return k / k.sum()


class PixelNorm(nn.Module):
    def forward(self, input):
        return input * torch.rsqrt(torch.mean(input ** 2, dim=1, keepdim=True) + 1e-8)


class _FirModule(nn.Module):

    def __init__(self, kernel, up, down, pad, ops):
        super().__init__()
        self.register_buffer("kernel", kernel)
        self.up, self.down, self.pad = up, down, pad
        self.ops = ops if ops is not None else cuda_ops()

    def forward(self, input):
        return self.ops.upfirdn2d(input, self.kernel, up=self.up, down=self.down, pad=self.pad)


class Upsample(_FirModule):
    def __init__(self, kernel, factor=2, ops=None):
        k = make_kernel(kernel) * (factor ** 2)
        p = k.shape[0] - factor
        super().__init__(k, factor, 1, ((p + 1) // 2 + factor - 1, p // 2), ops)
        self.factor = factor


class Downsample(_FirModule):
    def __init__(self, kernel, factor=2, ops=None):
        k = make_kernel(kernel)
        p = k.shape[0] - factor
        super().__init__(k, 1, factor, ((p + 1) // 2, p // 2), ops)
        self.factor = factor


class Blur(_FirModule):
    def __init__(self, kernel, pad, upsample_factor=1, ops=None):
        k = make_kernel(kernel)
        if upsample_factor > 1:
            k = k * (upsample_factor ** 2)
        super().__init__(k, 1, 1, pad, ops)


class EqualConv2d(nn.Module):
    def __init__(self, in_channel, out_channel, kernel_size, stride=1, padding=0, bias=True, ops=None):
        super().__init__()
        self.weight = nn.Parameter(torch.randn(out_channel, in_channel, kernel_size, kernel_size))
        self.scale = 1 / math.sqrt(in_channel * kernel_size ** 2)
        self.stride, self.padding = stride, padding
        self.bias = nn.Parameter(torch.zeros(out_channel)) if bias else None
        self.ops = ops if ops is not None else cuda_ops()

    scaler = None

    def forward(self, input, gain=1.0):
        w = self.scaler.get(self, input.dtype, gain) if self.scaler is not None and input.is_cuda else None
        if w is None:
            w = self.weight * (self.scale * gain)
        b = self.bias
        if w.dtype != input.dtype:
            w = w.to(input.dtype)
        if b is not None and b.dtype != input.dtype:
            b = b.to(input.dtype)
        return self.ops.conv2d(input, w, bias=b, stride=self.stride, padding=self.padding)

    def __repr__(self):
        return (f"{self.__class__.__name__}({self.weight.shape[1]}, {self.weight.shape[0]},"
                f" {self.weight.shape[2]}, stride={self.stride}, padding={self.padding})")


class EqualLinear(nn.Module):
    def __init__(self, in_dim, out_dim, bias=True, bias_init=0, lr_mul=1, activation=None, ops=None):
        super().__init__()
        self.weight = nn.Parameter(torch.randn(out_dim, in_dim).div_(lr_mul))
        self.bias = nn.Parameter(torch.zeros(out_dim).fill_(bias_init)) if bias else None
        self.activation = activation
        self.scale = (1 / math.sqrt(in_dim)) * lr_mul
        self.lr_mul = lr_mul
        self.ops = ops if ops is not None else cuda_ops()

    scaler = None

    def forward(self, input):
        w = self.scaler.get(self, input.dtype) if self.scaler is not None and input.is_cuda else None
        if w is None:
            w = self.weight * self.scale
        if self.activation:
            out = F.linear(input, w)
            return self.ops.fused_leaky_relu(out, self.bias * self.lr_mul)
        return F.linear(input, w, bias=self.bias * self.lr_mul)

    def __repr__(self):
        return f"{self.__class__.__name__}({self.weight.shape[1]}, {self.weight.shape[0]})"


class ScaledLeakyReLU(nn.Module):
    def __init__(self, negative_slope=0.2):
        super().__init__()
        self.negative_slope = negative_slope

    def forward(self, input):
        return F.leaky_relu(input, negative_slope=self.negative_slope) * math.sqrt(2)


class FusedLeakyReLU(nn.Module):

    def __init__(self, channel, negative_slope=0.2, scale=2 ** 0.5, ops=None):
        super().__init__()
        self.bias = nn.Parameter(torch.zeros(channel))
        self.negative_slope, self.scale = negative_slope, scale
        self.ops = ops if ops is not None else cuda_ops()

    def forward(self, input):
        bias = self.bias if input.dtype == torch.bfloat16 else self.bias.type(input.dtype)
        return self.ops.fused_leaky_relu(input, bias, self.negative_slope, self.scale)


class ModulatedConv2d(nn.Module):

    def __init__(self, in_channel, out_channel, kernel_size, style_dim, demodulate=True, upsample=False,
                 downsample=False, blur_kernel=[1, 3, 3, 1], normalize=False, ops=None):
        super().__init__()
        self.eps = 1e-8
        self.kernel_size, self.in_channel, self.out_channel = kernel_size, in_channel, out_channel
        self.upsample, self.downsample, self.normalize = upsample, downsample, normalize
        self.ops = ops if ops is not None else cuda_ops()
        if upsample:
            factor = 2
            p = (len(blur_kernel) - factor) - (kernel_size - 1)
            self.blur = Blur(blur_kernel, pad=((p + 1) // 2 + factor - 1, p // 2 + 1), upsample_factor=factor, ops=ops)
        if downsample:
            factor = 2
            p = (len(blur_kernel) - factor) + (kernel_size - 1)
            self.blur = Blur(blur_kernel, pad=((p + 1) // 2, p // 2), ops=ops)
        self.scale = 1 / math.sqrt(in_channel * kernel_size ** 2)
        self.padding = kernel_size // 2
        self.weight = nn.Parameter(torch.randn(1, out_channel, in_channel, kernel_size, kernel_size))
        self.modulation = EqualLinear(style_dim, in_channel, bias_init=1, ops=ops)
        self.demodulate = demodulate

    def __repr__(self):
        return (f"{self.__class__.__name__}({self.in_channel}, {self.out_channel}, {self.kernel_size}, "
                f"upsample={self.upsample}, downsample={self.downsample})")

    def conv_raw(self, input, style):
        style = self.modulation(style)
        plain = not (self.normalize or (input.dtype == torch.float16 and self.demodulate)) and not self.downsample
        if plain:
            return self.ops.modulated_conv2d(input, self.weight, style, self.scale, self.demodulate, self.upsample,
                                             self.padding, self.eps)
        return self._reference_formulation(input, style), None

    def forward(self, input, style, fuse_blur=True):
        raw, demod = self.conv_raw(input, style)
        if demod is not None:
            raw = self.ops.channel_scale(raw, demod)
        if self.upsample and fuse_blur:
            return self.blur(raw)
        return raw

    def _reference_formulation(self, input, style):
        batch, in_channel, height, width = input.shape
        weight = self.weight
        scale = self.scale
        if self.normalize or (input.dtype == torch.float16 and self.demodulate):
            style = style / torch.max(torch.abs(style))
            fan = torch.tensor(in_channel * weight.size(3) * weight.size(4), dtype=torch.float32)
            weight = scale * weight * torch.sqrt(1.0 / fan) / torch.amax(torch.abs(scale * weight), dim=(2, 3, 4), keepdims=True)
            scale = 1.0
        w = self.ops.modulated_weight(weight, style, scale, self.demodulate, transposed=self.upsample, eps=self.eps)
        w = w.type(input.dtype)
        x = input.reshape(1, batch * in_channel, height, width)
        if self.upsample:
            out = self.ops.conv_transpose2d(x, w, padding=0, stride=2, groups=batch)
        elif self.downsample:
            xb = self.blur(input)
            out = self.ops.conv2d(xb.reshape(1, batch * in_channel, xb.shape[2], xb.shape[3]), w, padding=0, stride=2,
                                  groups=batch)
        else:
            out = self.ops.conv2d(x, w, padding=self.padding, groups=batch)
        return out.view(batch, self.out_channel, out.shape[2], out.shape[3])


class NoiseInjection(nn.Module):
    def __init__(self):
        super().__init__()
        self.weight = nn.Parameter(torch.zeros(1))

    @staticmethod
    def sample(batch, height, width, like):
        return like.new_empty(batch, 1, height, width).normal_()

    def forward(self, image, noise=None):
        if noise is None:
            noise = self.sample(image.shape[0], image.shape[2], image.shape[3], image)
        return image + self.weight.type(image.dtype) * noise.type(image.dtype)


class ConstantInput(nn.Module):
    def __init__(self, channel, size=4):
        super().__init__()
        self.input = nn.Parameter(torch.randn(1, channel, size, size))
        self.size = size

    def forward(self, input):
        return self.input.repeat(input.shape[0], 1, 1, 1)


class StyledConv(nn.Module):

    def __init__(self, in_channel, out_channel, kernel_size, style_dim, upsample=False, blur_kernel=[1, 3, 3, 1],
                 demodulate=True, normalize=False, ops=None):
        super().__init__()
        self.conv = ModulatedConv2d(in_channel, out_channel, kernel_size, style_dim, upsample=upsample,
                                    blur_kernel=blur_kernel, demodulate=demodulate, normalize=normalize, ops=ops)
        self.noise = NoiseInjection()
        self.activate = FusedLeakyReLU(out_channel, ops=ops)
        self.ops = ops if ops is not None else cuda_ops()

    def forward(self, input, style, noise=None):
        act = self.activate
        raw, demod = self.conv.conv_raw(input, style)
        if self.conv.upsample:
            blur = self.conv.blur
            out_h = raw.shape[2] + blur.pad[0] + blur.pad[1] - blur.kernel.shape[0] + 1
            out_w = raw.shape[3] + blur.pad[0] + blur.pad[1] - blur.kernel.shape[1] + 1
            if noise is None:
                noise = NoiseInjection.sample(raw.shape[0], out_h, out_w, raw)
            return self.ops.blur_noise_bias_act(raw, blur.kernel, blur.pad, noise, self.noise.weight, act.bias,
                                                act.negative_slope, act.scale, row_scale=demod)
        if noise is None:
            noise = NoiseInjection.sample(raw.shape[0], raw.shape[2], raw.shape[3], raw)
        return self.ops.noise_bias_act(raw, noise, self.noise.weight, act.bias, act.negative_slope, act.scale,
                                       row_scale=demod)


class ToRGB(nn.Module):
    def __init__(self, in_channel, style_dim, upsample=True, blur_kernel=[1, 3, 3, 1], normalize=False, ops=None):
        super().__init__()
        if upsample:
            self.upsample = Upsample(blur_kernel, ops=ops)
        self.conv = ModulatedConv2d(in_channel, 3, 1, style_dim, demodulate=False, normalize=normalize, ops=ops)
        self.bias = nn.Parameter(torch.zeros(1, 3, 1, 1))

    def forward(self, input, style, skip=None):
        conv = self.conv
        up = self.upsample(skip) if skip is not None else None
        if not (conv.normalize or conv.downsample or conv.upsample or conv.demodulate):
            out, _ = conv.ops.modulated_conv2d(input, conv.weight, conv.modulation(style), conv.scale, False, False,
                                               conv.padding, conv.eps, bias=self.bias, skip=up)
            return out
        out = conv(input, style) + self.bias.type(input.dtype)
        if up is not None:
            out = out.float() + up
        return out


class ConvLayer(nn.Sequential):

    def __init__(self, in_channel, out_channel, kernel_size, downsample=False, blur_kernel=[1, 3, 3, 1], bias=True,
                 activate=True, ops=None):
        layers = []
        if downsample:
            factor = 2
            p = (len(blur_kernel) - factor) + (kernel_size - 1)
            layers.append(Blur(blur_kernel, pad=((p + 1) // 2, p // 2), ops=ops))
            stride, self.padding = 2, 0
        else:
            stride, self.padding = 1, kernel_size // 2
        layers.append(EqualConv2d(in_channel, out_channel, kernel_size, padding=self.padding, stride=stride,
                                  bias=bias and not activate, ops=ops))
        if activate:
            layers.append(FusedLeakyReLU(out_channel, ops=ops) if bias else ScaledLeakyReLU(0.2))
        super().__init__(*layers)


class ResBlock(nn.Module):
    def __init__(self, in_channel, out_channel, blur_kernel=[1, 3, 3, 1], downsample=True, ops=None):
        super().__init__()
        self.conv1 = ConvLayer(in_channel, in_channel, 3, ops=ops)
        self.conv2 = ConvLayer(in_channel, out_channel, 3, downsample=downsample, ops=ops)
        self.skip = ConvLayer(in_channel, out_channel, 1, downsample=downsample, activate=False, bias=False, ops=ops)

    def forward(self, input):
        act, skip_conv = self.conv2[-1], self.skip[-1]
        if (input.is_cuda and isinstance(act, FusedLeakyReLU) and getattr(act.ops, "name", None) == "sm_90a"
                and isinstance(skip_conv, EqualConv2d) and skip_conv.bias is None):
            inv = 1.0 / math.sqrt(2)
            main = self.conv1(input)
            for layer in list(self.conv2)[:-1]:
                main = layer(main)
            bias = act.bias if main.dtype == torch.bfloat16 else act.bias.type(main.dtype)
            main = act.ops.fused_leaky_relu(main, bias, act.negative_slope, act.scale * inv)
            side = input
            for layer in list(self.skip)[:-1]:
                side = layer(side)
            return main + skip_conv(side, gain=inv)
        return (self.conv2(self.conv1(input)) + self.skip(input)) / math.sqrt(2)


def channel_table(channel_multiplier):
    return {4: 512, 8: 512, 16: 512, 32: 512, 64: 256 * channel_multiplier, 128: 128 * channel_multiplier,
            256: 64 * channel_multiplier, 512: 32 * channel_multiplier, 1024: 16 * channel_multiplier}


class Generator(nn.Module):

    def __init__(self, size, style_dim, n_mlp, channel_multiplier=2, blur_kernel=[1, 3, 3, 1], lr_mlp=0.01,
                 num_fp16_res=0, run_fp32=True, ops=None):
        super().__init__()
        self.size, self.style_dim = size, style_dim
        self.style = nn.Sequential(PixelNorm(), *[EqualLinear(style_dim, style_dim, lr_mul=lr_mlp, activation="fused_lrelu", ops=ops)
                                                  for _ in range(n_mlp)])
        self.channels = channel_table(channel_multiplier)
        self.input = ConstantInput(self.channels[4])
        self.conv1 = StyledConv(self.channels[4], self.channels[4], 3, style_dim, blur_kernel=blur_kernel, ops=ops)
        self.to_rgb1 = ToRGB(self.channels[4], style_dim, upsample=False, ops=ops)
        self.log_size = int(math.log(size, 2))
        self.num_layers = (self.log_size - 2) * 2 + 1
        self.convs, self.upsamples, self.to_rgbs = nn.ModuleList(), nn.ModuleList(), nn.ModuleList()
        self.noises = nn.Module()
        for layer_idx in range(self.num_layers):
            res = (layer_idx + 5) // 2
            self.noises.register_buffer(f"noise_{layer_idx}", torch.randn(1, 1, 2 ** res, 2 ** res))
        in_channel = self.channels[4]
        for i in range(3, self.log_size + 1):
            mixed = i > self.log_size - num_fp16_res
            out_channel = self.channels[2 ** i]
            self.convs.append(StyledConv(in_channel, out_channel, 3, style_dim, upsample=True, blur_kernel=blur_kernel,
                                         normalize=mixed, ops=ops))
            self.convs.append(StyledConv(out_channel, out_channel, 3, style_dim, blur_kernel=blur_kernel,
                                         normalize=mixed, ops=ops))
            self.to_rgbs.append(ToRGB(out_channel, style_dim, normalize=False, ops=ops))
            in_channel = out_channel
        self.n_latent = self.log_size * 2 - 2
        self.num_fp16_res, self.run_fp32 = num_fp16_res, run_fp32
        self.channels_last = False
        self.act_dtype = torch.float32
        self.fuse_synthesis = True

    def ops_are_native(self):
        return getattr(self.conv1.ops, "name", None) == "sm_90a"

    def make_noise(self, batch_size=1):
        device = self.input.input.device
        noises = [torch.randn(batch_size, 1, 4, 4, device=device)]
        for i in range(3, self.log_size + 1):
            noises += [torch.randn(batch_size, 1, 2 ** i, 2 ** i, device=device) for _ in range(2)]
        return noises

    def batch_latent(self, n_latent):
        return self.style(torch.randn(n_latent, self.style_dim, device=self.input.input.device))

    def mean_latent(self, n_latent):
        return self.batch_latent(n_latent).mean(dim=0, keepdim=True)

    def get_latent(self, input):
        return self.style(input)

    def forward(self, styles, mapping_only=False, return_latents=False, inject_index=None, truncation=1,
                truncation_latent=None, input_is_latent=False, noise=None, randomize_noise=True):
        if not input_is_latent:
            styles = [self.style(s) for s in styles]
            if mapping_only:
                return styles
        if noise is None:
            noise = [None] * self.num_layers if randomize_noise else \
                [getattr(self.noises, f"noise_{i}") for i in range(self.num_layers)]
        if truncation < 1:
            styles = [truncation_latent + truncation * (styles[0] - truncation_latent), styles[0]]
        row_needs_grad = None
        if len(styles) < 2 or inject_index == self.n_latent:
            inject_index = self.n_latent
            latent = styles[0].unsqueeze(1).repeat(1, inject_index, 1) if styles[0].ndim < 3 else styles[0]
        else:
            if inject_index is None:
                inject_index = random.randint(1, self.n_latent - 1)
            latent = torch.cat([styles[0].unsqueeze(1).repeat(1, inject_index, 1),
                                styles[1].unsqueeze(1).repeat(1, self.n_latent - inject_index, 1)], 1)
            row_needs_grad = [styles[0].requires_grad] * inject_index + [styles[1].requires_grad] * (self.n_latent - inject_index)

        if self.channels_last and self.fuse_synthesis and self.ops_are_native():
            from ..op import styled_fused
            if styled_fused.fusable(self, latent, self.act_dtype):
                image = styled_fused.synthesis(self, latent, noise, self.act_dtype, row_needs_grad)
                return (image, latent) if return_latents else (image, None)
        x0 = self.input(latent)
        if self.channels_last:
            x0 = x0.contiguous(memory_format=torch.channels_last)
        out = self.conv1(x0, latent[:, 0], noise=noise[0])
        skip = self.to_rgb1(out, latent[:, 1])
        i = 1
        for j, (up, conv, n_up, n_conv, to_rgb) in enumerate(
                zip(self.convs[::2], self.convs[1::2], noise[1::2], noise[2::2], self.to_rgbs), 3):
            half = j > self.log_size - self.num_fp16_res and not self.run_fp32
            out = out.type(torch.float16 if half else torch.float32)
            out = up(out, latent[:, i], noise=n_up)
            out = conv(out, latent[:, i + 1], noise=n_conv)
            skip = to_rgb(out, latent[:, i + 2], skip)
            i += 2
        return (skip, latent) if return_latents else (skip, None)
```

gangealing_b200/training/perceptual.py:

```python
import torch
import torch.nn as nn


_VGG16_CFG = [64, 64, "M", 128, 128, "M", 256, 256, 256, "M", 512, 512, 512, "M", 512, 512, 512]
_SLICE_ENDS = (4, 9, 16, 23, 30)
_CHNS = (64, 128, 256, 512, 512)


def _vgg16_features():
    layers, c_in = [], 3
    for v in _VGG16_CFG:
        if v == "M":
            layers.append(nn.MaxPool2d(kernel_size=2, stride=2))
        else:
            layers += [nn.Conv2d(c_in, v, kernel_size=3, padding=1), nn.ReLU(inplace=False)]
            c_in = v
    return layers


class VGG16Slices(nn.Module):

    def __init__(self):
        super().__init__()
        feats = _vgg16_features()
        starts = (0,) + _SLICE_ENDS[:-1]
        for k, (a, b) in enumerate(zip(starts, _SLICE_ENDS), 1):
            seq = nn.Sequential()
            for idx in range(a, b):
                seq.add_module(str(idx), feats[idx])
            setattr(self, "slice%d" % k, seq)
        self.N_slices = 5
        for p in self.parameters():
            p.requires_grad = False

    def slices(self):
        return [getattr(self, "slice%d" % k) for k in range(1, self.N_slices + 1)]

    def load_features_state_dict(self, state_dict, strict=True):
        own = {}
        for k, seq in enumerate(self.slices(), 1):
            for idx, layer in seq.named_children():
                for name, _ in layer.named_parameters():
                    own["%s.%s" % (idx, name)] = "slice%d.%s.%s" % (k, idx, name)
        unexpected = [k for k in state_dict if k not in own]
        if strict and unexpected:
            raise RuntimeError("unexpected VGG16 feature keys (the reference slices stop at relu5_3): %s" % unexpected[:4])
        return self.load_state_dict({own[k]: v for k, v in state_dict.items() if k in own}, strict=strict)

    def forward(self, x, ops=None):
        outs = []
        slices = self.slices()
        pooled = None
        for k, s in enumerate(slices):
            if ops is None or not x.is_cuda:
                x = s(x)
            else:
                layers = list(s.children())
                nxt = list(slices[k + 1].children()) if k + 1 < len(slices) else []
                pool_next = bool(nxt) and isinstance(nxt[0], nn.MaxPool2d) and _is_2x2_pool(nxt[0]) and hasattr(ops, "bias_relu_pool")
                i = 0
                if pooled is not None:
                    x, pooled, i = pooled, None, 1
                while i < len(layers):
                    m = layers[i]
                    if isinstance(m, nn.Conv2d) and i + 1 < len(layers) and isinstance(layers[i + 1], nn.ReLU):
                        x = nn.functional.conv2d(x, m.weight, None, m.stride, m.padding, m.dilation, m.groups)
                        bias = m.bias.float() if m.bias.dtype != torch.float32 else m.bias
                        if i + 2 == len(layers) and pool_next and ops.bias_relu_pool_supported(x):
                            x, pooled = ops.bias_relu_pool(x, bias)
                        else:
                            x = ops.fused_leaky_relu(x, bias, 0.0, 1.0)
                        i += 2
                    else:
                        x = m(x)
                        i += 1
            outs.append(x)
        return outs


def _is_2x2_pool(m):
    def pair(v):
        return tuple(v) if isinstance(v, (tuple, list)) else (v, v)
    return (pair(m.kernel_size) == (2, 2) and pair(m.stride) == (2, 2) and pair(m.padding) == (0, 0) and pair(m.dilation) == (1, 1)
            and not m.ceil_mode and not m.return_indices)


class ScalingLayer(nn.Module):
    def __init__(self):
        super().__init__()
        self.register_buffer("shift", torch.tensor([-.030, -.088, -.188])[None, :, None, None])
        self.register_buffer("scale", torch.tensor([.458, .448, .450])[None, :, None, None])

    def forward(self, inp):
        return (inp - self.shift) / self.scale


class NetLinLayer(nn.Module):

    def __init__(self, chn_in, chn_out=1, use_dropout=False):
        super().__init__()
        layers = [nn.Dropout()] if use_dropout else []
        layers += [nn.Conv2d(chn_in, chn_out, 1, stride=1, padding=0, bias=False)]
        self.model = nn.Sequential(*layers)

    def forward(self, x):
        return self.model(x)


class PerceptualLoss(nn.Module):

    def __init__(self, divisor=18.0, lpips=False, use_dropout=True, pretrained_weights=None, ops=None):
        super().__init__()
        self.ops = ops
        self.scaling_layer = ScalingLayer()
        self.net = VGG16Slices()
        self.lpips = lpips
        self.L = 5
        if lpips:
            for k, c in enumerate(_CHNS):
                setattr(self, "lin%d" % k, NetLinLayer(c, use_dropout=use_dropout))
            self.lins = nn.ModuleList([getattr(self, "lin%d" % k) for k in range(self.L)])
        if pretrained_weights is not None:
            sd = pretrained_weights if isinstance(pretrained_weights, dict) else \
                torch.load(pretrained_weights, map_location="cpu")
            self.net.load_features_state_dict(sd, strict=True)
        self.divisor = divisor
        self.eval()
        for p in self.parameters():
            p.requires_grad = False


    def forward(self, in0, in1):
        cl = torch.channels_last if in0.is_cuda else torch.contiguous_format
        dt = self.net.slice1[0].weight.dtype
        ops = self.ops
        if ops is None:
            from ..opset import cuda_ops
            ops = cuda_ops()
        native = ops if getattr(ops, "name", None) == "sm_90a" else None
        if native is not None and in0.is_cuda and in0.shape == in1.shape and hasattr(ops, "feature_distance_stacked"):
            feats = self.net(self.scaling_layer(torch.cat([in0, in1], 0)).to(dt).contiguous(memory_format=cl), native)
            val = 0
            for k, f in enumerate(feats):
                w = self.lins[k].model[-1].weight.reshape(-1) if self.lpips else None
                val = val + ops.feature_distance_stacked(f, w)
            return val / self.divisor
        f0 = self.net(self.scaling_layer(in0).to(dt).contiguous(memory_format=cl), native)
        f1 = self.net(self.scaling_layer(in1).to(dt).contiguous(memory_format=cl), native)
        val = 0
        for k, (a, b) in enumerate(zip(f0, f1)):
            w = self.lins[k].model[-1].weight.reshape(-1) if self.lpips else None
            val = val + ops.feature_distance(a, b, w)
        return val / self.divisor


def get_perceptual_loss(device, seed=0, ops=None, kind="vgg_ssl", pretrained_weights=None, lpips_weights=None):
    g = torch.random.get_rng_state()
    torch.manual_seed(seed)
    if kind == "vgg_ssl":
        loss = PerceptualLoss(divisor=18.0, lpips=False, pretrained_weights=pretrained_weights, ops=ops)
    elif kind == "lpips":
        loss = PerceptualLoss(divisor=1.0, lpips=True, pretrained_weights=pretrained_weights, ops=ops)
        if lpips_weights is not None:
            sd = lpips_weights if isinstance(lpips_weights, dict) else torch.load(lpips_weights, map_location="cpu")
            loss.load_state_dict(sd, strict=False)
    else:
        raise NotImplementedError(kind)
    torch.random.set_rng_state(g)
    loss = loss.to(device)
    if torch.device(device).type == "cuda":
        loss = loss.to(memory_format=torch.channels_last)
    return loss
```

include/gg_b200.h:

```cpp
#ifndef GG_B200_H_
#define GG_B200_H_

#include <stdint.h>

#ifdef __cplusplus
extern "C" {
#endif

#define GG_API __attribute__((visibility("default")))

enum { GG_F32 = 0, GG_F16 = 1, GG_BF16 = 2, GG_F64 = 3 };

enum {
  GG_OK = 0,
  GG_ERR_BAD_ARG = -1,
  GG_ERR_UNSUPPORTED = -2,
  GG_ERR_CUDA = -3
};

enum { GG_PAD_ZEROS = 0, GG_PAD_BORDER = 1, GG_PAD_REFLECTION = 2 };

GG_API int gg_version(void);
GG_API const char* gg_last_error(void);
GG_API int gg_sm_count(void);

GG_API int gg_fused_bias_act(void* out, const void* x, const void* bias, const void* ref, int dtype,
                             int act, int grad, float alpha, float scale, int64_t size_x,
                             int64_t step_b, int64_t size_b, void* stream);

GG_API int gg_noise_bias_act(void* out, const void* x, const void* noise, const float* noise_weight,
                             const float* bias, const float* row_scale, int dtype, float alpha, float scale,
                             int64_t N, int64_t C, int64_t HW, void* stream);

GG_API int64_t gg_channel_scale_workspace(int64_t rows, int64_t HW);
GG_API int gg_channel_scale(void* out, float* row_dot, void* workspace, const void* x, const void* y,
                            const float* s, int dtype, int64_t rows, int64_t HW, void* stream);

GG_API int64_t gg_bias_act_backward_workspace(int64_t N, int64_t C, int64_t HW);
GG_API int gg_bias_act_backward(void* gx, float* grad_bias, void* workspace, const void* g,
                                const void* out, int dtype, float alpha, float scale, int64_t N,
                                int64_t C, int64_t HW, void* stream);

GG_API int gg_upfirdn2d(void* out, const void* in, const float* kernel, int dtype, int64_t major,
                        int in_h, int in_w, int kernel_h, int kernel_w, int up_x, int up_y,
                        int down_x, int down_y, int pad_x0, int pad_x1, int pad_y0, int pad_y1,
                        void* stream);

GG_API int gg_blur_noise_bias_act(void* out, const void* in, const float* kernel, const void* noise,
                                  const float* noise_weight, const float* bias,
                                  const float* row_scale, int dtype, int64_t N, int64_t C, int in_h,
                                  int in_w, int kernel_h, int kernel_w, int pad_x0, int pad_x1,
                                  int pad_y0, int pad_y1, int act, float alpha, float scale,
                                  void* stream);

GG_API int64_t gg_mipmap_pyramid_elems(int64_t planes, int hs, int ws, int extra_levels);
GG_API int gg_mipmap_build(float* pyramid, const void* src, int dtype, int64_t planes, int hs, int ws,
                           int extra_levels, void* stream);
GG_API int gg_mipmap_build_backward(float* grad_src, float* grad_pyramid, int64_t planes, int hs, int ws,
                                    int extra_levels, void* stream);
GG_API int gg_mipmap_warp_forward(void* out, float* levels_out, const void* src, const float* pyramid,
                                  const float* grid, int dtype, int64_t N, int C, int hs, int ws, int ho,
                                  int wo, int extra_levels, float max_level, float min_level,
                                  int padding_mode, void* stream);
GG_API int gg_mipmap_warp_backward(float* grad_src, float* grad_pyramid, float* grad_grid,
                                   const void* grad_out, const void* src, const float* pyramid,
                                   const float* grid, int dtype, int64_t N, int C, int hs, int ws, int ho,
                                   int wo, int extra_levels, float max_level, float min_level,
                                   int padding_mode, void* stream);
GG_API int gg_warp_sample_indices(int32_t* indices, const float* grid, int64_t N, int hs, int ws, int ho, int wo,
                                  float max_level, float min_level, int padding_mode, void* stream);
GG_API int gg_mipmap_warp_lerp_forward(void* out, float* grid_out, const void* src, const float* pyramid, const float* base,
                                       int64_t base_stride, const float* target, const float* alphas, int T, int dtype,
                                       int64_t N, int C, int hs, int ws, int ho, int wo, int extra_levels, float max_level,
                                       float min_level, int padding_mode, void* stream);
GG_API int gg_mipmap_warp_lerp_mean(float* acc, const void* src, const float* pyramid, const float* base, int64_t base_stride,
                                    const float* target, const float* alphas, int T, int dtype, int64_t N, int C, int hs,
                                    int ws, int ho, int wo, int extra_levels, float max_level, float min_level,
                                    int padding_mode, int accumulate, void* stream);

GG_API int gg_flow_compose_forward(float* delta_flow, float* flow, const float* low_flow, const float* mask,
                                   const float* identity_flow, const float* base_warp, const float* alpha,
                                   int64_t N, int H, int W, int S, void* stream);
GG_API int gg_flow_compose_backward(float* grad_mask, float* grad_low_flow, float* grad_base_warp,
                                    const float* grad_delta, const float* grad_flow, const float* low_flow,
                                    const float* mask, const float* identity_flow, const float* base_warp,
                                    const float* alpha, int64_t N, int H, int W, int S, void* stream);

GG_API int64_t gg_splat2d_workspace(int64_t N, int C, int H, int W);
GG_API int gg_splat2d_forward(float* out, void* workspace, const float* input, const float* coordinates,
                              const float* values, const float* sigma, int64_t N, int64_t P, int C, int H,
                              int W, int soft_normalize, void* stream);

GG_API int64_t gg_splat_composite_grid_workspace(int64_t T_chunk, int64_t N, int R, int has_alpha);
GG_API int gg_splat_composite_grid(unsigned char* out, void* workspace, int64_t workspace_bytes, const float* images,
                                   const float* points, const float* colors, const float* alpha, float sigma,
                                   float opacity, int64_t T, int64_t N, int64_t P, int C, int R, int nrow, int padding,
                                   int colors_n, int alpha_n, void* stream);

GG_API int gg_stn_sample_forward(void* out, float* grid_out, float* delta_out, float* levels_out, const void* src,
                                 const float* pyramid, const float* theta, const float* low, const float* mask,
                                 const float* identity, const float* alpha, int mode, int dtype, int64_t N, int C,
                                 int hs, int ws, int ho, int wo, int lh, int lw, int s, int extra_levels,
                                 float max_level, float min_level, int padding_mode, void* stream);

GG_API int gg_modconv_wsq(float* wsq, const float* weight, int O, int I, int kk, void* stream);
GG_API int gg_modconv_demod(float* demod, const float* wsq, const float* style, float scale, float eps, int B,
                            int O, int I, void* stream);
GG_API int gg_modconv_demod_batched(int layers, float* const* demod, const float* const* wsq, const float* const* style,
                                    const float* scale, const int* O, const int* I, float eps, int B, void* stream);
GG_API int gg_modconv_modulate(float* out, const float* weight, const float* style, const float* demod,
                               float scale, int B, int O, int I, int kk, int transposed, void* stream);

GG_API int gg_noise_bias_act_nhwc(void* out, const void* x, const float* noise, const float* noise_weight,
                                  const float* bias, const float* row_scale, int dtype, float alpha, float scale,
                                  int64_t N, int C, int64_t HW, void* stream);
GG_API int64_t gg_nhwc_rowwise_workspace(int64_t N, int C, int64_t HW);
GG_API int gg_channel_scale_nhwc(void* out, float* row_dot, void* workspace, const void* x, const void* y,
                                 const float* s, int dtype, int64_t N, int C, int64_t HW, void* stream);
GG_API int gg_bias_act_backward_nhwc(void* gx, float* grad_bias, void* workspace, const void* g,
                                     const void* out_saved, int dtype, float alpha, float scale, int64_t N, int C,
                                     int64_t HW, void* stream);
GG_API int64_t gg_blur_nhwc_workspace(int dtype, int64_t N, int C, int in_h, int in_w, int kernel_h, int kernel_w,
                                      int pad_x0, int pad_x1, int pad_y0, int pad_y1);
GG_API int gg_blur_nhwc(void* out, void* out2, const void* in, const float* kernel, const float* noise,
                        const float* noise_weight, const float* bias, const float* row_scale, const float* scale2,
                        const void* mul, float* row_dot, void* workspace, int dtype, int64_t N, int C, int in_h,
                        int in_w, int kernel_h, int kernel_w, int separable, int pad_x0, int pad_x1, int pad_y0,
                        int pad_y1, int mode, int act, float alpha, float scale, void* stream);
GG_API int gg_blur_nhwc_mask(void* mask, void* out2, const void* in, const float* kernel, const float* noise,
                             const float* noise_weight, const float* bias, const float* row_scale, const float* scale2,
                             int dtype, int64_t N, int C, int in_h, int in_w, int kernel_h, int kernel_w, int separable,
                             int pad_x0, int pad_x1, int pad_y0, int pad_y1, int act, float alpha, float scale,
                             void* stream);

GG_API int gg_styled_tail_nhwc(void* out, void* xs, float* rgb, const void* raw, const float* noise,
                               const float* noise_weight, const float* bias, const float* demod, const float* s_next,
                               const float* wm, const float* rgb_bias, const float* skip, int dtype, int act,
                               float alpha, float scale, int64_t N, int C, int64_t HW, void* stream);
GG_API int64_t gg_styled_tail_backward_workspace(int dtype, int64_t N, int C, int64_t HW);
GG_API int gg_styled_tail_backward_nhwc(void* g_raw, float* d_s_next, float* d_demod, float* d_wm, void* workspace,
                                        const void* g_xs, const float* g_rgb, const void* out_saved, const void* raw,
                                        const float* s_next, const float* demod, const float* wm, int dtype,
                                        float alpha, float scale, int64_t N, int C, int64_t HW, int64_t reduce_pitch,
                                        void* stream);
GG_API int gg_styled_tail_mask_nhwc(void* mask, void* xs, float* rgb, const void* raw, const float* noise,
                                    const float* noise_weight, const float* bias, const float* demod,
                                    const float* s_next, const float* wm, const float* rgb_bias, const float* skip,
                                    int dtype, int act, float alpha, float scale, int64_t N, int C, int64_t HW,
                                    void* stream);
GG_API int gg_styled_tail_backward_mask_nhwc(void* g_raw, const void* g_xs, const float* g_rgb, const void* mask,
                                             const float* s_next, const float* demod, const float* wm, int dtype,
                                             float alpha, float scale, int64_t N, int C, int64_t HW, void* stream);

GG_API int64_t gg_to_rgb_nhwc_workspace(int64_t N, int C, int64_t HW);
GG_API int gg_to_rgb_nhwc_forward(float* out, const float* x, const float* wm, const float* bias, const float* skip,
                                  int64_t N, int C, int64_t HW, void* stream);
GG_API int gg_to_rgb_nhwc_backward(float* gx, float* gwm, void* workspace, const float* g, const float* x,
                                   const float* wm, int64_t N, int C, int64_t HW, void* stream);


GG_API int64_t gg_feature_distance_workspace(int64_t N, int C, int64_t HW);
GG_API int gg_feature_distance_forward(float* out, void* workspace, const void* f0, const void* f1,
                                       const float* weight, int dtype, int64_t N, int C, int64_t HW, float eps,
                                       void* stream);
GG_API int gg_feature_distance_backward(void* g0, void* g1, const float* grad_out, const void* f0, const void* f1,
                                        const float* weight, int dtype, int64_t N, int C, int64_t HW, float eps,
                                        void* stream);

GG_API int gg_bias_relu_pool_nhwc_forward(void* y, void* pooled, const void* raw, const float* bias, int dtype, int64_t N,
                                          int C, int H, int W, void* stream);
GG_API int gg_bias_relu_pool_nhwc_backward(void* grad_raw, const void* grad_y, const void* grad_pooled, const void* y,
                                           int dtype, int64_t N, int C, int H, int W, void* stream);

GG_API int gg_tent_downsample_forward(float* out, const float* in, const float* taps_h, const float* taps_v, int64_t N,
                                      int C, int in_h, int in_w, int stride, void* stream);
GG_API int gg_tent_downsample_backward(float* grad_in, const float* grad_out, const float* taps_h, const float* taps_v,
                                       int64_t N, int C, int in_h, int in_w, int stride, void* stream);

GG_API int64_t gg_nn_argmin_workspace(int64_t N, int64_t P);
GG_API int gg_nn_argmin(int64_t* index, void* workspace, const float* grid, const float* points, int64_t N, int64_t P, int HW,
                        void* stream);
GG_API int gg_track_points_lerp(int64_t* track, int64_t* centers, const float* base, const float* target, const float* alphas,
                                const float* points, int T, int64_t N, int64_t P, int H, int W, int patch, void* stream);
GG_API int gg_splat2d_lookup_forward(float* out, float* points_out, void* workspace, const float* input, const float* grid,
                                     const float* query, const float* values, const float* sigma, int64_t N, int64_t P,
                                     int C, int H, int W, int grid_h, int grid_w, float unnorm_k, float unnorm_m,
                                     int soft_normalize, void* stream);

GG_API int gg_tv_per_sample(float* out, const float* flow, int64_t N, int H, int W, void* stream);
GG_API int64_t gg_pck_transfer_workspace(int64_t B, int64_t P, int F);
GG_API int gg_pck_transfer(int64_t* counts, float* est_points, int64_t* nn_index, void* workspace, const float* points,
                           const float* gt_points, const float* visible, const float* thresh, const float* alphas,
                           const float* matrix_src, const float* matrix_dst, const float* delta_src, const float* identity,
                           const float* grid_dst, int64_t B, int64_t P, int A, int S, int F, int grid_h, int grid_w,
                           void* stream);

GG_API int64_t gg_laplacian_blend_workspace(int64_t N, int C, int H, int W, int levels, int backward);
GG_API int gg_laplacian_blend_forward(float* out, void* workspace, const float* img0, const float* img1, const float* mask,
                                      const float* taps, int64_t N, int C, int H, int W, int levels, int width, void* stream);
GG_API int gg_laplacian_blend_backward(float* grad_img0, float* grad_img1, float* grad_mask, void* workspace,
                                       const float* grad_out, const float* img0, const float* img1, const float* mask,
                                       const float* taps, int64_t N, int C, int H, int W, int levels, int width,
                                       void* stream);

GG_API int gg_adam_ema_step(const void* table, const int* block_tensor, const int* block_chunk, int blocks, int chunk,
                            float* state, double beta1, double beta2, double eps, double ema_decay, void* stream);
GG_API int64_t gg_tv_loss_workspace(int64_t N, int H, int W);
GG_API int gg_tv_loss_forward(float* out, void* workspace, const float* flow, int64_t N, int H, int W, void* stream);
GG_API int gg_tv_loss_backward(float* grad_flow, const float* grad_out, const float* flow, int64_t N, int H, int W,
                               void* stream);

GG_API int gg_scale_cast_multi(const void* table, const int* block_tensor, const int* block_chunk, int blocks, int chunk,
                               void* stream);

GG_API int gg_batch_gram(double* gram, double* mean, const float* w, const int64_t* batch_offsets, int64_t B, int D,
                         void* stream);

GG_API int gg_flow_image_grid(unsigned char* out, void* workspace, const float* flow, int64_t N, int H, int W, int nrow,
                              int padding, void* stream);
GG_API int gg_image_grid(unsigned char* out, const float* images, const float* ranges, int64_t N, int H, int W, int nrow,
                         int padding, void* stream);
GG_API int gg_cluster_accumulate(float* sums, int64_t* counts, float* keep, const float* images, const int64_t* sel,
                                 int64_t N, int S, int K, int C, int H, int W, int64_t stride_n, int64_t stride_flip,
                                 int64_t stride_head, int64_t stride_c, int64_t stride_h, int64_t stride_w, int n_keep,
                                 void* stream);

#ifdef __cplusplus
}
#endif
#endif
```

Measured before the change: 496.7.

## Store leaky-ReLU sign as bitmask and fuse residual add into trunk bias-act

Adds a bias+leaky-ReLU kernel that saves a 1-bit-per-element sign mask instead of the full activation, plus a backward that reads the mask. It also fuses the residual-block skip add into the activation and folds the skip-blur backward plus gradient add into one blur pass (mode 4). These are applied to StyleGAN trunk layers and the perceptual network ReLUs. The aim is less saved-activation memory traffic and fewer elementwise passes, at the cost of new code paths that only run when C is a multiple of 32 and tensors are aligned.

```diff
diff --git a/gangealing_b200/_lib.py b/gangealing_b200/_lib.py
--- a/gangealing_b200/_lib.py
+++ b/gangealing_b200/_lib.py
@@ -41,6 +41,8 @@
     "gg_nhwc_rowwise_workspace": (_L, [_L, _I, _L]),
     "gg_channel_scale_nhwc": (_I, [_P] * 6 + [_I, _L, _I, _L, _P]),
     "gg_bias_act_backward_nhwc": (_I, [_P] * 5 + [_I, _F, _F, _L, _I, _L, _P]),
+    "gg_bias_act_mask_nhwc": (_I, [_P] * 5 + [_I, _F, _F, _L, _I, _L, _P]),
+    "gg_bias_act_backward_mask_nhwc": (_I, [_P] * 5 + [_I, _F, _F, _L, _I, _L, _P]),
     "gg_blur_nhwc_workspace": (_L, [_I, _L] + [_I] * 9),
     "gg_blur_nhwc": (_I, [_P] * 12 + [_I, _L] + [_I] * 12 + [_F, _F, _P]),
     "gg_blur_nhwc_mask": (_I, [_P] * 9 + [_I, _L] + [_I] * 11 + [_F, _F, _P]),
diff --git a/gangealing_b200/csrc/common.cuh b/gangealing_b200/csrc/common.cuh
--- a/gangealing_b200/csrc/common.cuh
+++ b/gangealing_b200/csrc/common.cuh
@@ -80,6 +80,9 @@
   static __device__ __forceinline__ float to_f(__nv_bfloat16 v) { return __bfloat162float(v); }
   static __device__ __forceinline__ __nv_bfloat16 from_f(float v) { return __float2bfloat16_rn(v); }
 };
+
+template <typename T>
+__device__ __forceinline__ float round_to(float v) { return Cvt<T>::to_f(Cvt<T>::from_f(v)); }
 
 template <typename T> struct alignas(16) Vec16 {
   static constexpr int N = 16 / sizeof(T);
diff --git a/gangealing_b200/csrc/nhwc.cu b/gangealing_b200/csrc/nhwc.cu
--- a/gangealing_b200/csrc/nhwc.cu
+++ b/gangealing_b200/csrc/nhwc.cu
@@ -79,7 +79,12 @@
     float sv[V];
 #pragma unroll
     for (int k = 0; k < V; ++k) sv[k] = (MODE == 0) ? __ldg(s + n * cv * V + cq * V + k) : 1.f;
-    const bool has_y = (MODE == 1) || y != nullptr;
+    const bool has_y = (MODE != 0) || y != nullptr;
+    const uint32_t* mw = reinterpret_cast<const uint32_t*>(y) + n * hw * (cv * V >> 5);
+    auto load_y = [&](int64_t p_, int64_t off_) -> uint4 {
+      if (MODE == 2) return make_uint4(sign_load<V>(mw + p_ * (cv * V >> 5), cq), 0u, 0u, 0u);
+      return has_y ? ldg_stream16(y + off_) : make_uint4(0u, 0u, 0u, 0u);
+    };
     auto body = [&](const uint4 xr, const uint4 yr, int64_t off) {
       float xf[V], yf[V], o[V];
       ChanVec<T>::unpack(xr, xf);
@@ -89,14 +94,16 @@
         if (MODE == 0) {
           o[k] = xf[k] * sv[k];
           if (has_y) acc[k] = fmaf(xf[k], yf[k], acc[k]);
-        } else {
+        } else if (MODE == 1) {
           o[k] = (yf[k] > 0.f ? xf[k] : xf[k] * alpha) * gain;
           acc[k] += o[k];
+        } else {
+          o[k] = (((yr.x >> k) & 1u) ? xf[k] : xf[k] * alpha) * gain;
+          acc[k] += o[k];
         }
       }
       *reinterpret_cast<uint4*>(out + off) = ChanVec<T>::pack(o);
     };
-    const uint4 zero = make_uint4(0u, 0u, 0u, 0u);
     int64_t p = p0 + pl;
     for (; p + 3 * lanes_p < p1; p += 4 * lanes_p) {
       uint4 xv[4], yv[4];
@@ -107,14 +114,14 @@
         xv[u] = ldg_stream16(x + off[u]);
       }
 #pragma unroll
-      for (int u = 0; u < 4; ++u) yv[u] = has_y ? ldg_stream16(y + off[u]) : zero;
+      for (int u = 0; u < 4; ++u) yv[u] = load_y(p + u * lanes_p, off[u]);
 #pragma unroll
       for (int u = 0; u < 4; ++u) body(xv[u], yv[u], off[u]);
     }
     for (; p < p1; p += lanes_p) {
       const int64_t off = ((n * hw + p) * cv + cq) * V;
       const uint4 xv = ldg_stream16(x + off);
-      const uint4 yv = has_y ? ldg_stream16(y + off) : zero;
+      const uint4 yv = load_y(p, off);
       body(xv, yv, off);
     }
   }
@@ -439,7 +446,8 @@
         if (okc[j]) mnext[j] = __ldg(reinterpret_cast<const uint4*>(mul + mo + static_cast<int64_t>(j) * p.c));
     }
   };
-  if (MODE == 2 && mul) { fetch_mul(-3 + 3); }
+  constexpr bool MUL = MODE == 2 || MODE == 4;
+  if (MUL && mul) { fetch_mul(-3 + 3); }
 
   float hwin[SEP ? 4 : 1][COLS][V];
   float rwin[SEP ? 1 : 4][COLS + 3][V];
@@ -461,7 +469,7 @@
 #pragma unroll
       for (int j = 0; j < COLS; ++j) nzc[rr][j] = nzn[rr][j];
     if (FUSED && noise && it + 1 < n_stage_iters) fetch_noise(it + 1);
-    if (MODE == 2 && mul && it + 1 < n_stage_iters) {
+    if (MUL && mul && it + 1 < n_stage_iters) {
 #pragma unroll
       for (int rr = 0; rr < kRY; ++rr) {
         const int ro = (it + 1) * kRY + rr - 3;
@@ -477,7 +485,7 @@
     const T* st = tiles + stage * G::STAGE_ELEMS;
 #pragma unroll
     for (int rr = 0; rr < kRY; ++rr, ++r_in, ocur += row_stride) {
-      if (MODE == 2 && mul) {
+      if (MUL && mul) {
 #pragma unroll
         for (int j = 0; j < COLS; ++j) mcur[j] = mnext[j];
         fetch_mul(r_in - 3 + 1);
@@ -562,6 +570,14 @@
               for (int k = 0; k < V; ++k) a4[k] *= rq[k];
               *reinterpret_cast<uint4*>(out + ooff) = ChanVec<T>::pack(a4);
             }
+          } else if (MODE == 4) {
+            if (okc[j]) {
+              float mf[V];
+              ChanVec<T>::unpack(mcur[j], mf);
+#pragma unroll
+              for (int k = 0; k < V; ++k) a4[k] = __fadd_rn(round_to<T>(a4[k]), mf[k]);
+              *reinterpret_cast<uint4*>(out + ooff) = ChanVec<T>::pack(a4);
+            }
           } else {
             if (okc[j]) *reinterpret_cast<uint4*>(out + ooff) = ChanVec<T>::pack(a4);
           }
@@ -690,9 +706,13 @@
                   (rowwise_nhwc_kernel<T_, 0><<<g, kT, smem, st>>>(static_cast<T_*>(out), partial, static_cast<const T_*>(x),
                                                                  dst ? static_cast<const T_*>(y) : nullptr, s, alpha, gain,
                                                                  cv, HW, chunk, K)));
+  } else if (mode == 1) {
+    GG_DISPATCH_T(dtype, "nhwc rowwise",
+                  (rowwise_nhwc_kernel<T_, 1><<<g, kT, smem, st>>>(static_cast<T_*>(out), partial, static_cast<const T_*>(x),
+                                                                 static_cast<const T_*>(y), s, alpha, gain, cv, HW, chunk, K)));
   } else {
     GG_DISPATCH_T(dtype, "nhwc rowwise",
-                  (rowwise_nhwc_kernel<T_, 1><<<g, kT, smem, st>>>(static_cast<T_*>(out), partial, static_cast<const T_*>(x),
+                  (rowwise_nhwc_kernel<T_, 2><<<g, kT, smem, st>>>(static_cast<T_*>(out), partial, static_cast<const T_*>(x),
                                                                  static_cast<const T_*>(y), s, alpha, gain, cv, HW, chunk, K)));
   }
   GG_CHECK_LAUNCH("nhwc rowwise launch");
@@ -716,6 +736,13 @@
                               int dtype, float alpha, float scale, int64_t N, int C, int64_t HW, void* stream) {
   if (!out_saved) return fail(GG_ERR_BAD_ARG, "bias_act_backward_nhwc: null saved output");
   return launch_rowwise(1, gx, grad_bias, workspace, g, out_saved, nullptr, dtype, alpha, scale, N, C, HW, false, stream);
+}
+
+int gg_bias_act_backward_mask_nhwc(void* gx, float* grad_bias, void* workspace, const void* g, const void* mask, int dtype,
+                                   float alpha, float scale, int64_t N, int C, int64_t HW, void* stream) {
+  if (!mask) return fail(GG_ERR_BAD_ARG, "bias_act_backward_mask_nhwc: null mask");
+  if (C % 32 != 0) return fail(GG_ERR_UNSUPPORTED, "bias_act_backward_mask_nhwc: C must be a multiple of 32");
+  return launch_rowwise(2, gx, grad_bias, workspace, g, mask, nullptr, dtype, alpha, scale, N, C, HW, false, stream);
 }
 
 int64_t gg_to_rgb_nhwc_workspace(int64_t N, int C, int64_t HW) { return 3 * gg_nhwc_rowwise_workspace(N, C, HW); }
@@ -860,7 +887,7 @@
   static DeviceOnce configured;
   if (configured.needed()) {
     cudaError_t e = cudaSuccess;
-    const void* kernels[12] = {reinterpret_cast<const void*>(blur_nhwc_kernel<T, 0, true>),
+    const void* kernels[14] = {reinterpret_cast<const void*>(blur_nhwc_kernel<T, 0, true>),
                               reinterpret_cast<const void*>(blur_nhwc_kernel<T, 0, false>),
                               reinterpret_cast<const void*>(blur_nhwc_kernel<T, 1, true, false>),
                               reinterpret_cast<const void*>(blur_nhwc_kernel<T, 1, false, false>),
@@ -871,8 +898,10 @@
                               reinterpret_cast<const void*>(blur_nhwc_kernel<T, 3, true, true>),
                               reinterpret_cast<const void*>(blur_nhwc_kernel<T, 3, false, true>),
                               reinterpret_cast<const void*>(blur_nhwc_kernel<T, 2, true>),
-                              reinterpret_cast<const void*>(blur_nhwc_kernel<T, 2, false>)};
-    for (int i = 0; i < 12 && e == cudaSuccess; ++i)
+                              reinterpret_cast<const void*>(blur_nhwc_kernel<T, 2, false>),
+                              reinterpret_cast<const void*>(blur_nhwc_kernel<T, 4, true>),
+                              reinterpret_cast<const void*>(blur_nhwc_kernel<T, 4, false>)};
+    for (int i = 0; i < 14 && e == cudaSuccess; ++i)
       e = cudaFuncSetAttribute(kernels[i], cudaFuncAttributeMaxDynamicSharedMemorySize, static_cast<int>(smem));
     if (e != cudaSuccess) return cuda_fail(e, "blur_nhwc smem opt-in");
     configured.done();
@@ -893,6 +922,7 @@
     else { if (separable) GG_BLUR(1, true, false); else GG_BLUR(1, false, false); }
   }
   else if (mode == 2) { if (separable) GG_BLUR(2, true, false); else GG_BLUR(2, false, false); }
+  else if (mode == 4) { if (separable) GG_BLUR(4, true, false); else GG_BLUR(4, false, false); }
   else { if (separable) GG_BLUR(0, true, false); else GG_BLUR(0, false, false); }
 #undef GG_BLUR
   GG_CHECK_LAUNCH("blur_nhwc launch");
@@ -912,7 +942,8 @@
                  int pad_x0, int pad_x1, int pad_y0, int pad_y1, int mode, int act, float alpha, float scale, void* stream) {
   if (N < 0 || C < 0 || in_h < 1 || in_w < 1) return fail(GG_ERR_BAD_ARG, "blur_nhwc: bad shape");
   if (kernel_h < 1 || kernel_w < 1 || kernel_h > 4 || kernel_w > 4) return fail(GG_ERR_UNSUPPORTED, "blur_nhwc: filter must be <= 4x4");
-  if (mode < 0 || mode > 2) return fail(GG_ERR_BAD_ARG, "blur_nhwc: mode must be 0 (blur), 1 (fused tail) or 2 (adjoint epilogue)");
+  if (mode < 0 || mode > 4 || mode == 3)
+    return fail(GG_ERR_BAD_ARG, "blur_nhwc: mode must be 0 (blur), 1 (fused tail), 2 (adjoint epilogue) or 4 (blur + add)");
   if (act != 1 && act != 3) return fail(GG_ERR_UNSUPPORTED, "blur_nhwc: act must be 1 or 3");
   if (dtype != GG_F32 && dtype != GG_BF16) return fail(GG_ERR_UNSUPPORTED, "blur_nhwc: dtype %d not supported (fp32 or bf16)", dtype);
   if (N == 0 || C == 0) return GG_OK;
@@ -920,8 +951,10 @@
   if (mode == 1 ? (!out && !out2) : !out) return fail(GG_ERR_BAD_ARG, "blur_nhwc: null output");
   if (mode != 1 && out2) return fail(GG_ERR_BAD_ARG, "blur_nhwc: out2 belongs to the fused tail (mode 1)");
   if (mode == 2 && row_dot && (!mul || !workspace)) return fail(GG_ERR_BAD_ARG, "blur_nhwc: row_dot needs `mul` and a workspace");
+  if (mode == 4 && !mul) return fail(GG_ERR_BAD_ARG, "blur_nhwc: mode 4 needs the addend `mul`");
+  if (mode == 4 && !aligned16(mul)) return fail(GG_ERR_BAD_ARG, "blur_nhwc: `mul` must be 16-byte aligned");
   if (N > 65535) return fail(GG_ERR_UNSUPPORTED, "blur_nhwc: batch > 65535");
-  if (mode == 0) { noise = nullptr; noise_weight = nullptr; bias = nullptr; row_scale = nullptr; scale2 = nullptr; }
+  if (mode == 0 || mode == 4) { noise = nullptr; noise_weight = nullptr; bias = nullptr; row_scale = nullptr; scale2 = nullptr; }
   GG_DISPATCH_T(dtype, "blur_nhwc",
                 return launch_blur<T_>(out, out2, in, kernel, noise, noise_weight, bias, row_scale, scale2, mul, row_dot,
                                        workspace, N, C, in_h, in_w, kernel_h, kernel_w, separable, pad_x0, pad_x1, pad_y0,
diff --git a/gangealing_b200/csrc/trunk.cu b/gangealing_b200/csrc/trunk.cu
--- /dev/null
+++ b/gangealing_b200/csrc/trunk.cu
@@ -0,0 +1,98 @@
+#include "common.cuh"
+
+namespace gg {
+namespace {
+
+constexpr int kT = 256;
+
+template <typename T, bool RES>
+__global__ void __launch_bounds__(kT)
+bias_act_mask_nhwc_kernel(T* __restrict__ out, uint32_t* __restrict__ mask, const T* __restrict__ x,
+                          const T* __restrict__ res, const float* __restrict__ bias, float alpha, float gain,
+                          int64_t n_vec, int cv) {
+  constexpr int V = ChanVec<T>::V;
+  constexpr int L = 32 / V;
+  const unsigned gmask = ((1u << L) - 1u) << (threadIdx.x & 31 & ~(L - 1));
+  const int64_t base = (static_cast<int64_t>(blockIdx.x) * 4) * kT + threadIdx.x;
+  uint4 xv[4], rv[4];
+#pragma unroll
+  for (int u = 0; u < 4; ++u) {
+    const int64_t v = base + static_cast<int64_t>(u) * kT;
+    if (v < n_vec) {
+      xv[u] = ldg_stream16(x + v * V);
+      if (RES) rv[u] = ldg_stream16(res + v * V);
+    }
+  }
+#pragma unroll
+  for (int u = 0; u < 4; ++u) {
+    const int64_t v = base + static_cast<int64_t>(u) * kT;
+    if (v < n_vec) {
+      const int cq = n_vec <= 0xffffffffLL ? static_cast<int>(static_cast<unsigned>(v) % static_cast<unsigned>(cv))
+                                           : static_cast<int>(v % cv);
+      float xf[V], o[V];
+      ChanVec<T>::unpack(xv[u], xf);
+#pragma unroll
+      for (int q = 0; q < V / 4; ++q) {
+        const float4 b = bias ? __ldg(reinterpret_cast<const float4*>(bias) + cq * (V / 4) + q) : make_float4(0.f, 0.f, 0.f, 0.f);
+        const float bb[4] = {b.x, b.y, b.z, b.w};
+#pragma unroll
+        for (int k = 0; k < 4; ++k) {
+          const float t = __fadd_rn(fmaf(xf[4 * q + k], 1.f, bb[k]), 0.f);
+          o[4 * q + k] = (t > 0.f ? t : t * alpha) * gain;
+        }
+      }
+      if (mask) {
+        const uint32_t word = sign_word<V>(sign_bits<T>(o), cq, gmask);
+        if ((cq & (L - 1)) == 0) mask[v / L] = word;
+      }
+      if (RES) {
+        float rf[V];
+        ChanVec<T>::unpack(rv[u], rf);
+#pragma unroll
+        for (int k = 0; k < V; ++k) o[k] = __fadd_rn(round_to<T>(o[k]), rf[k]);
+      }
+      stg_stream16(out + v * V, ChanVec<T>::pack(o));
+    }
+  }
+}
+
+}
+}
+
+using namespace gg;
+
+extern "C" {
+
+int gg_bias_act_mask_nhwc(void* out, void* mask, const void* x, const void* res, const float* bias, int dtype, float alpha,
+                          float scale, int64_t N, int C, int64_t HW, void* stream) {
+  if (N < 0 || C < 0 || HW < 0) return fail(GG_ERR_BAD_ARG, "bias_act_mask_nhwc: negative size");
+  if (dtype != GG_F32 && dtype != GG_BF16) return fail(GG_ERR_UNSUPPORTED, "bias_act_mask_nhwc: dtype %d not supported", dtype);
+  if (C % 32 != 0) return fail(GG_ERR_UNSUPPORTED, "bias_act_mask_nhwc: C must be a multiple of 32");
+  const int64_t numel = N * HW * C;
+  if (numel == 0) return GG_OK;
+  if (!out || !x) return fail(GG_ERR_BAD_ARG, "bias_act_mask_nhwc: null tensor");
+  if (!aligned16(out) || !aligned16(x) || !aligned16(res) || !aligned16(bias))
+    return fail(GG_ERR_BAD_ARG, "bias_act_mask_nhwc: out, x, res and bias must be 16-byte aligned");
+  if (!aligned16(mask)) return fail(GG_ERR_BAD_ARG, "bias_act_mask_nhwc: mask must be 16-byte aligned");
+  const int V = dtype == GG_BF16 ? 8 : 4;
+  const int64_t n_vec = numel / V;
+  const int64_t grid = (n_vec + 4 * kT - 1) / (4 * kT);
+  if (grid > 0x7fffffffLL) return fail(GG_ERR_BAD_ARG, "bias_act_mask_nhwc: tensor too large");
+  auto st = static_cast<cudaStream_t>(stream);
+  const unsigned g = static_cast<unsigned>(grid);
+  uint32_t* m = static_cast<uint32_t*>(mask);
+  if (res) {
+    GG_DISPATCH_T(dtype, "bias_act_mask_nhwc",
+                  (bias_act_mask_nhwc_kernel<T_, true><<<g, kT, 0, st>>>(static_cast<T_*>(out), m, static_cast<const T_*>(x),
+                                                                       static_cast<const T_*>(res), bias, alpha, scale,
+                                                                       n_vec, C / V)));
+  } else {
+    GG_DISPATCH_T(dtype, "bias_act_mask_nhwc",
+                  (bias_act_mask_nhwc_kernel<T_, false><<<g, kT, 0, st>>>(static_cast<T_*>(out), m, static_cast<const T_*>(x),
+                                                                        nullptr, bias, alpha, scale, n_vec, C / V)));
+  }
+  GG_CHECK_LAUNCH("bias_act_mask_nhwc launch");
+  return GG_OK;
+}
+
+}
diff --git a/gangealing_b200/op/nhwc.py b/gangealing_b200/op/nhwc.py
--- a/gangealing_b200/op/nhwc.py
+++ b/gangealing_b200/op/nhwc.py
@@ -69,11 +69,12 @@
     out2 = empty() if (mode == 1 and want_out2) else None
     nz = noise_plane(noise, n, out_h, out_w) if mode == 1 else None
     dot = ws = None
-    if mode == 2 and want_dot:
+    if mode == 4 or (mode == 2 and want_dot):
         if (mul is None or mul.shape != (n, c, out_h, out_w) or mul.dtype != x.dtype or not mul.is_contiguous(memory_format=CL)
                 or not _lib.aligned16(mul)):
-            raise RuntimeError("blur (adjoint epilogue): `mul` must be a 16-byte-aligned channels-last tensor of the output's "
+            raise RuntimeError("blur (modes 2 and 4): `mul` must be a 16-byte-aligned channels-last tensor of the output's "
                                "shape and dtype")
+    if mode == 2 and want_dot:
         dot = torch.empty((n, c), dtype=torch.float32, device=x.device)
         nbytes = lib.gg_blur_nhwc_workspace(code, n, c, in_h, in_w, kh, kw, pad[0], pad[1], pad[2], pad[3])
         ws = torch.empty(max(1, nbytes // 4), dtype=torch.float32, device=x.device)
@@ -90,7 +91,7 @@
     else:
         rc = lib.gg_blur_nhwc(_lib.ptr(out), _lib.ptr(out2), x.data_ptr(), taps.data_ptr(), _lib.ptr(nz),
                               _lib.ptr(nw), _lib.ptr(b), _lib.ptr(rs),
-                              _lib.ptr(s2), _lib.ptr(mul if dot is not None else None), _lib.ptr(dot), _lib.ptr(ws),
+                              _lib.ptr(s2), _lib.ptr(mul if (dot is not None or mode == 4) else None), _lib.ptr(dot), _lib.ptr(ws),
                               code, n, c, in_h, in_w, kh, kw, sep, pad[0], pad[1],
                               pad[2], pad[3], mode, act, negative_slope, gain, _lib.stream())
     _lib.check(rc, "gg_blur_nhwc_mask" if want_mask else "gg_blur_nhwc")
@@ -126,6 +127,41 @@
     rc = lib.gg_bias_act_backward_nhwc(gx.data_ptr(), _lib.ptr(grad_bias), _lib.ptr(ws), g.data_ptr(), out_saved.data_ptr(),
                                        _lib.dtype_code(out_saved), negative_slope, gain, n, c, h * w, _lib.stream())
     _lib.check(rc, "gg_bias_act_backward_nhwc")
+    return gx, grad_bias
+
+
+def mask_ok(t):
+    return rowwise_ok(t) and t.shape[1] % 32 == 0
+
+
+def bias_act_mask(x, res, bias, want_mask, negative_slope, gain):
+    n, c, h, w = x.shape
+    _activation_like(x, x, "bias_act_mask", "x")
+    _activation_like(res, x, "bias_act_mask", "res")
+    out = torch.empty_like(x)
+    mask = sign_mask_empty(n, c, h, w, x.device) if want_mask else None
+    b = _f32(bias, c)
+    rc = _lib.load().gg_bias_act_mask_nhwc(out.data_ptr(), _lib.ptr(mask), x.data_ptr(), _lib.ptr(res), _lib.ptr(b),
+                                           _lib.dtype_code(x), negative_slope, gain, n, c, h * w, _lib.stream())
+    _lib.check(rc, "gg_bias_act_mask_nhwc")
+    return out, mask
+
+
+def bias_act_backward_mask(g, mask, negative_slope, gain, want_bias_grad):
+    n, h, w, words = mask.shape
+    c = 32 * words
+    _activation_like(g, g, "bias_act_backward_mask", "g")
+    if g.shape != (n, c, h, w):
+        raise RuntimeError("bias_act_backward_mask: the gradient's shape does not match the mask's")
+    lib = _lib.load()
+    gx = torch.empty_like(g)
+    grad_bias = ws = None
+    if want_bias_grad:
+        grad_bias = torch.empty(c, dtype=torch.float32, device=g.device)
+        ws = torch.empty(max(1, lib.gg_nhwc_rowwise_workspace(n, c, h * w) // 4), dtype=torch.float32, device=g.device)
+    rc = lib.gg_bias_act_backward_mask_nhwc(gx.data_ptr(), _lib.ptr(grad_bias), _lib.ptr(ws), g.data_ptr(), mask.data_ptr(),
+                                            _lib.dtype_code(g), negative_slope, gain, n, c, h * w, _lib.stream())
+    _lib.check(rc, "gg_bias_act_backward_mask_nhwc")
     return gx, grad_bias
 
 
diff --git a/gangealing_b200/op/trunk.py b/gangealing_b200/op/trunk.py
--- /dev/null
+++ b/gangealing_b200/op/trunk.py
@@ -0,0 +1,75 @@
+import torch
+from torch.autograd import Function
+from torch.autograd.function import once_differentiable
+
+from .. import _lib
+from . import nhwc
+from .upfirdn2d import grad_pad, upfirdn2d_raw
+
+
+def supported(x, res=None):
+    return (x.is_cuda and nhwc.mask_ok(x)
+            and (res is None or (res.shape == x.shape and res.dtype == x.dtype and nhwc.mask_ok(res))))
+
+
+class _BiasActMask(Function):
+    @staticmethod
+    def forward(ctx, x, res, bias, negative_slope, gain):
+        out, mask = nhwc.bias_act_mask(x, res, bias, True, negative_slope, gain)
+        ctx.save_for_backward(mask)
+        ctx.cfg = (negative_slope, gain, x.dtype, bias.dtype if bias is not None else None)
+        return out
+
+    @staticmethod
+    @once_differentiable
+    def backward(ctx, g):
+        (mask,) = ctx.saved_tensors
+        negative_slope, gain, dtype, bias_dtype = ctx.cfg
+        want_x, want_res, want_bias = ctx.needs_input_grad[:3]
+        gx = grad_bias = None
+        if want_x or want_bias:
+            gc = g.contiguous(memory_format=torch.channels_last)
+            if gc.dtype != dtype:
+                gc = gc.to(dtype)
+            if not nhwc.mask_ok(gc):
+                gc = gc.clone(memory_format=torch.channels_last)
+            gx, grad_bias = nhwc.bias_act_backward_mask(gc, mask, negative_slope, gain, want_bias)
+            if grad_bias is not None:
+                grad_bias = grad_bias.to(bias_dtype)
+        return gx, (g if want_res else None), grad_bias, None, None
+
+
+def bias_act(x, bias, negative_slope=0.2, gain=2 ** 0.5, res=None):
+    if torch.is_grad_enabled() and any(t is not None and t.requires_grad for t in (x, res, bias)):
+        return _BiasActMask.apply(x, res, bias, negative_slope, gain)
+    out, _ = nhwc.bias_act_mask(x, res, bias, False, negative_slope, gain)
+    return out
+
+
+class _SkipBlurFork(Function):
+    @staticmethod
+    def forward(ctx, x, kernel, pad):
+        out = upfirdn2d_raw(x, kernel, (1, 1), (1, 1), pad)
+        kh, kw = kernel.shape
+        ctx.save_for_backward(kernel)
+        ctx.g_pad = grad_pad(x.shape[2], x.shape[3], out.shape[2], out.shape[3], kh, kw, (1, 1), (1, 1), pad)
+        return x.view_as(x), out
+
+    @staticmethod
+    @once_differentiable
+    def backward(ctx, g_main, g_blur):
+        (kernel,) = ctx.saved_tensors
+        if g_blur is None:
+            return g_main, None, None
+        flipped = _lib.flipped_filter(kernel)
+        if (g_main is not None and nhwc.blur_ok(g_blur, *flipped.shape) and g_main.dtype == g_blur.dtype
+                and g_main.is_contiguous(memory_format=torch.channels_last) and _lib.aligned16(g_main)):
+            return nhwc.blur(g_blur, flipped, ctx.g_pad, mode=4, mul=g_main)[0], None, None
+        g_x = upfirdn2d_raw(g_blur, flipped, (1, 1), (1, 1), ctx.g_pad)
+        return (g_x if g_main is None else g_main + g_x), None, None
+
+
+def skip_blur_fork(x, kernel, pad):
+    if torch.is_grad_enabled() and x.requires_grad:
+        return _SkipBlurFork.apply(x, kernel, pad)
+    return x, upfirdn2d_raw(x, kernel, (1, 1), (1, 1), pad)
diff --git a/gangealing_b200/stylegan2/networks.py b/gangealing_b200/stylegan2/networks.py
--- a/gangealing_b200/stylegan2/networks.py
+++ b/gangealing_b200/stylegan2/networks.py
@@ -127,6 +127,10 @@
 
     def forward(self, input):
         bias = self.bias if input.dtype == torch.bfloat16 else self.bias.type(input.dtype)
+        if getattr(self.ops, "name", None) == "sm_90a":
+            from ..op import trunk
+            if trunk.supported(input):
+                return trunk.bias_act(input, bias, self.negative_slope, self.scale)
         return self.ops.fused_leaky_relu(input, bias, self.negative_slope, self.scale)
 
 
@@ -300,16 +304,24 @@
         act, skip_conv = self.conv2[-1], self.skip[-1]
         if (input.is_cuda and isinstance(act, FusedLeakyReLU) and getattr(act.ops, "name", None) == "sm_90a"
                 and isinstance(skip_conv, EqualConv2d) and skip_conv.bias is None):
+            from ..op import trunk
             inv = 1.0 / math.sqrt(2)
-            main = self.conv1(input)
+            x, side = input, input
+            skip_layers = list(self.skip)[:-1]
+            if len(skip_layers) == 1 and isinstance(skip_layers[0], Blur):
+                blur = skip_layers[0]
+                x, side = trunk.skip_blur_fork(input, blur.kernel, (blur.pad[0], blur.pad[1], blur.pad[0], blur.pad[1]))
+                skip_layers = []
+            for layer in skip_layers:
+                side = layer(side)
+            side = skip_conv(side, gain=inv)
+            main = self.conv1(x)
             for layer in list(self.conv2)[:-1]:
                 main = layer(main)
             bias = act.bias if main.dtype == torch.bfloat16 else act.bias.type(main.dtype)
-            main = act.ops.fused_leaky_relu(main, bias, act.negative_slope, act.scale * inv)
-            side = input
-            for layer in list(self.skip)[:-1]:
-                side = layer(side)
-            return main + skip_conv(side, gain=inv)
+            if trunk.supported(main, side):
+                return trunk.bias_act(main, bias, act.negative_slope, act.scale * inv, res=side)
+            return act.ops.fused_leaky_relu(main, bias, act.negative_slope, act.scale * inv) + side
         return (self.conv2(self.conv1(input)) + self.skip(input)) / math.sqrt(2)
 
 
diff --git a/gangealing_b200/training/perceptual.py b/gangealing_b200/training/perceptual.py
--- a/gangealing_b200/training/perceptual.py
+++ b/gangealing_b200/training/perceptual.py
@@ -51,6 +51,9 @@
         outs = []
         slices = self.slices()
         pooled = None
+        masked = getattr(ops, "name", None) == "sm_90a"
+        if masked:
+            from ..op import trunk
         for k, s in enumerate(slices):
             if ops is None or not x.is_cuda:
                 x = s(x)
@@ -68,6 +71,8 @@
                         bias = m.bias.float() if m.bias.dtype != torch.float32 else m.bias
                         if i + 2 == len(layers) and pool_next and ops.bias_relu_pool_supported(x):
                             x, pooled = ops.bias_relu_pool(x, bias)
+                        elif masked and trunk.supported(x):
+                            x = trunk.bias_act(x, bias, 0.0, 1.0)
                         else:
                             x = ops.fused_leaky_relu(x, bias, 0.0, 1.0)
                         i += 2
diff --git a/include/gg_b200.h b/include/gg_b200.h
--- a/include/gg_b200.h
+++ b/include/gg_b200.h
@@ -120,6 +120,10 @@
 GG_API int gg_bias_act_backward_nhwc(void* gx, float* grad_bias, void* workspace, const void* g,
                                      const void* out_saved, int dtype, float alpha, float scale, int64_t N, int C,
                                      int64_t HW, void* stream);
+GG_API int gg_bias_act_mask_nhwc(void* out, void* mask, const void* x, const void* res, const float* bias, int dtype,
+                                 float alpha, float scale, int64_t N, int C, int64_t HW, void* stream);
+GG_API int gg_bias_act_backward_mask_nhwc(void* gx, float* grad_bias, void* workspace, const void* g, const void* mask,
+                                          int dtype, float alpha, float scale, int64_t N, int C, int64_t HW, void* stream);
 GG_API int64_t gg_blur_nhwc_workspace(int dtype, int64_t N, int C, int in_h, int in_w, int kernel_h, int kernel_w,
                                       int pad_x0, int pad_x1, int pad_y0, int pad_y1);
 GG_API int gg_blur_nhwc(void* out, void* out2, const void* in, const float* kernel, const float* noise,
```

Result: faster. 504.5, median of 6 (+1.6%).
